# Ecogenomics/CheckM

Measured on NVIDIA H100. Metric: genomes/hour, higher is better.
Workload: dtype int16 (SSV) / u8 (MSV) / int16 (Viterbi) / f32 (Forward, domain definition)

## Files before the change

checkm_b200/csrc/fwdback_blk.cuh:

```cuda
#pragma once
#include "device_utils.cuh"
#include "engine.hpp"
#include "fwdback.cuh"

namespace ckm {

constexpr int BLK_LOOKAHEAD_MAXQ = 16;

template <int Q, bool TSMEM>
struct BlkModel {
  int M;
  const float *rfb;
  const float4 *tsm;
  float4 t0[TSMEM ? 1 : Q], t1[TSMEM ? 1 : Q];
  int lane;
  __device__ __forceinline__ float4 T0(int q) const { return TSMEM ? tsm[q * 32 + lane] : t0[TSMEM ? 0 : q]; }
  __device__ __forceinline__ float4 T1(int q) const { return TSMEM ? tsm[(Q + q) * 32 + lane] : t1[TSMEM ? 0 : q]; }
};

template <int Q, bool TSMEM>
__device__ __forceinline__ void blk_model_load(BlkModel<Q, TSMEM> &bm, const ModelScalars &ms, const float4 *tfb, const float *rfb,
                                               float4 *tsm, int lane) {
  bm.M = ms.M; bm.lane = lane;
  bm.rfb = rfb + ms.blk_off * 32 * KPAD + lane;
  bm.tsm = tsm;
  const float4 *src = tfb + ms.blk_off * 32 * 2;
  if (TSMEM) {
    __syncwarp();
    for (int q = 0; q < Q; ++q) { tsm[q * 32 + lane] = __ldg(src + (q * 32 + lane) * 2); tsm[(Q + q) * 32 + lane] = __ldg(src + (q * 32 + lane) * 2 + 1); }
    __syncwarp();
  } else {
#pragma unroll
    for (int q = 0; q < Q; ++q) { bm.t0[TSMEM ? 0 : q] = __ldg(src + (q * 32 + lane) * 2); bm.t1[TSMEM ? 0 : q] = __ldg(src + (q * 32 + lane) * 2 + 1); }
  }
}

template <int Q, bool TSMEM, bool FULL, bool STORE_D = true>
__device__ __forceinline__ float forward_blk(const BlkModel<Q, TSMEM> &bm, const uint8_t *__restrict__ res, int L, const Specials sp,
                                             float *xmx, float *full) {
  const int lane = bm.lane;
  float Mx[Q], Ix[Q], Dx[Q];
#pragma unroll
  for (int q = 0; q < Q; ++q) { Mx[q] = 0.0f; Ix[q] = 0.0f; Dx[q] = 0.0f; }
  if (FULL) {
#pragma unroll
    for (int z = 0; z < 3 * Q; ++z) full[z * 32 + lane] = 0.0f;
  }
  float xE = 0.0f, xN = 1.0f, xJ = 0.0f, xB = sp.nmove, xC = 0.0f, totscale = 0.0f;
  if (xmx != nullptr && lane == 0) { xmx[X_E] = xE; xmx[X_N] = xN; xmx[X_J] = xJ; xmx[X_B] = xB; xmx[X_C] = xC; xmx[X_SCALE] = 1.0f; }
  constexpr bool LA = (Q <= BLK_LOOKAHEAD_MAXQ);
  float ecur[Q];
  int xnext;
  if (LA) {
    const float *rp = bm.rfb + (size_t)((L >= 1) ? __ldg(res) : 0) * Q * 32;
#pragma unroll
    for (int q = 0; q < Q; ++q) ecur[q] = __ldg(rp + q * 32);
    xnext = (L >= 2) ? __ldg(res + 1) : 0;
  } else xnext = (L >= 1) ? __ldg(res) : 0;
  for (int i = 1; i <= L; ++i) {
    float enext[LA ? Q : 1];
    {
      const float *rp = bm.rfb + (size_t)xnext * Q * 32;
      if (LA) {
#pragma unroll
        for (int q = 0; q < Q; ++q) enext[LA ? q : 0] = __ldg(rp + q * 32);
        xnext = (i + 2 <= L) ? __ldg(res + i + 1) : 0;
      } else {
#pragma unroll
        for (int q = 0; q < Q; ++q) ecur[q] = __ldg(rp + q * 32);
        xnext = (i + 1 <= L) ? __ldg(res + i) : 0;
      }
    }
    float pm_in = __shfl_up_sync(0xffffffffu, Mx[Q - 1], 1), pi_in = __shfl_up_sync(0xffffffffu, Ix[Q - 1], 1), pd_in = __shfl_up_sync(0xffffffffu, Dx[Q - 1], 1);
    if (lane == 0) { pm_in = 0.0f; pi_in = 0.0f; pd_in = 0.0f; }
    float md[Q], esum = 0.0f;
#pragma unroll
    for (int q = Q - 1; q >= 0; --q) {
      const float4 t0 = bm.T0(q), t1 = bm.T1(q);
      const float pm = (q > 0) ? Mx[q - 1] : pm_in, pi = (q > 0) ? Ix[q - 1] : pi_in, pd = (q > 0) ? Dx[q - 1] : pd_in;
      float sv = xB * t0.x;
      sv += pm * t0.y;
      sv += pi * t0.z;
      sv += pd * t0.w;
      sv *= ecur[q];
      const float nI = Mx[q] * t1.y + Ix[q] * t1.z;
      md[q] = sv * t1.x;
      Mx[q] = sv; Ix[q] = nI;
      esum += sv;
    }
    float Bb = 0.0f, Tb = 1.0f;
#pragma unroll
    for (int q = 0; q < Q; ++q) { const float tdd = bm.T1(q).w; Bb = md[q] + Bb * tdd; Tb *= tdd; }
    float Bs = Bb, Ts = Tb;
#pragma unroll
    for (int o = 1; o < 32; o <<= 1) {
      const float Bl = __shfl_up_sync(0xffffffffu, Bs, o), Tl = __shfl_up_sync(0xffffffffu, Ts, o);
      if (lane >= o) { Bs = Bs + Bl * Ts; Ts = Ts * Tl; }
    }
    float d = __shfl_up_sync(0xffffffffu, Bs, 1);
    if (lane == 0) d = 0.0f;
#pragma unroll
    for (int q = 0; q < Q; ++q) {
      const bool in = (lane * Q + q + 1) <= bm.M;
      Dx[q] = in ? d : 0.0f;
      esum += Dx[q];
      d = md[q] + d * bm.T1(q).w;
    }
    xE = warp_sum_float(esum);
    xN = xN * sp.nloop;
    xC = (xC * sp.nloop) + (xE * sp.emove);
    xJ = (xJ * sp.nloop) + (xE * sp.eloop);
    xB = (xJ * sp.nmove) + (xN * sp.nmove);
    float scale = 1.0f;
    if (xE > 1.0e4f) {
      scale = xE;
      const float inv = __fdiv_rn(1.0f, xE);
      xN = __fdiv_rn(xN, xE); xC = __fdiv_rn(xC, xE); xJ = __fdiv_rn(xJ, xE); xB = __fdiv_rn(xB, xE);
#pragma unroll
      for (int q = 0; q < Q; ++q) { Mx[q] *= inv; Dx[q] *= inv; Ix[q] *= inv; }
      totscale += (float)log((double)xE);
      xE = 1.0f;
    }
    if (FULL) {
      float *fr = full + (size_t)i * 3 * Q * 32 + lane;
#pragma unroll
      for (int q = 0; q < Q; ++q) { fr[q * 32] = Mx[q]; if (STORE_D) fr[(Q + q) * 32] = Dx[q]; fr[(2 * Q + q) * 32] = Ix[q]; }
    }
    if (xmx != nullptr && lane == 0) {
      float *xr = xmx + (size_t)i * X_NX;
      xr[X_E] = xE; xr[X_N] = xN; xr[X_J] = xJ; xr[X_B] = xB; xr[X_C] = xC; xr[X_SCALE] = scale;
    }
    if (LA) {
#pragma unroll
      for (int q = 0; q < Q; ++q) ecur[q] = enext[LA ? q : 0];
    }
  }
  return totscale + (float)log((double)(xC * sp.nmove));
}

__device__ __forceinline__ void prefetch_l2(const void *p) { asm volatile("prefetch.global.L2 [%0];" ::"l"(p)); }
template <int Q, bool TSMEM, int MODE>
__device__ __forceinline__ void backward_blk(const BlkModel<Q, TSMEM> &bm, const uint8_t *__restrict__ res, int L, const Specials sp,
                                             const float *fxmx, float *bxmx, float *full) {
  const int lane = bm.lane, M = bm.M;
  float Mx[Q], Ix[Q], Dx[Q];
#pragma unroll
  for (int q = 0; q < Q; ++q) { Mx[q] = 0.0f; Ix[q] = 0.0f; Dx[q] = 0.0f; }
  float xC = 0.0f, xE = 0.0f, xJ = 0.0f, xN = 0.0f, xB = 0.0f;
  constexpr bool LA = (Q <= BLK_LOOKAHEAD_MAXQ);
  float ecur[Q];
#pragma unroll
  for (int q = 0; q < Q; ++q) ecur[q] = 0.0f;
  int xnext = (L >= 1) ? __ldg(res + L - 1) : 0;
  for (int i = L; i >= 0; --i) {
    float enext[LA ? Q : 1];
    if (LA) {
      const float *rp = bm.rfb + (size_t)xnext * Q * 32;
#pragma unroll
      for (int q = 0; q < Q; ++q) enext[LA ? q : 0] = __ldg(rp + q * 32);
      xnext = (i >= 2) ? __ldg(res + i - 2) : 0;
    } else if (i < L) {
      const float *rp = bm.rfb + (size_t)xnext * Q * 32;
#pragma unroll
      for (int q = 0; q < Q; ++q) ecur[q] = __ldg(rp + q * 32);
      xnext = (i >= 1) ? __ldg(res + i - 1) : 0;
    }
    if (MODE == 2 && i >= 3) {
      const float *fr = full + (size_t)(i - 2) * 3 * Q * 32;
      if (lane < Q) { prefetch_l2(fr + lane * 32); prefetch_l2(fr + (2 * Q + lane) * 32); }
    }
    float em[Q];
    if (i == L) {
      xC = sp.nmove; xE = xC * sp.emove; xB = 0.0f; xJ = 0.0f; xN = 0.0f;
#pragma unroll
      for (int q = 0; q < Q; ++q) em[q] = 0.0f;
    } else {
      float part = 0.0f;
#pragma unroll
      for (int q = 0; q < Q; ++q) { em[q] = Mx[q] * ecur[q]; part += em[q] * bm.T0(q).x; }
      xB = warp_sum_float(part);
      xC = xC * sp.nloop;
      xJ = (xB * sp.nmove) + (xJ * sp.nloop);
      xN = (xB * sp.nmove) + (xN * sp.nloop);
      xE = (xC * sp.emove) + (xJ * sp.eloop);
    }
    const float s = (i >= 1) ? fxmx[(size_t)i * X_NX + X_SCALE] : 1.0f;
    if (i >= 1) {
      const float inv = (s > 1.0f) ? __fdiv_rn(1.0f, s) : 1.0f;
      float em_next = __shfl_down_sync(0xffffffffu, em[0], 1);
      float4 tn_next;
      {
        const float4 mine = bm.T0(0);
        tn_next.x = 0.0f;
        tn_next.y = __shfl_down_sync(0xffffffffu, mine.y, 1); tn_next.z = __shfl_down_sync(0xffffffffu, mine.z, 1); tn_next.w = __shfl_down_sync(0xffffffffu, mine.w, 1);
      }
      if (lane == 31) { em_next = 0.0f; tn_next.y = 0.0f; tn_next.z = 0.0f; tn_next.w = 0.0f; }
      float cb[Q];
      float Bb = 0.0f, Tb = 1.0f;
#pragma unroll
      for (int q = Q - 1; q >= 0; --q) {
        const int k = lane * Q + q + 1;
        const float mnext = (q < Q - 1) ? em[q + 1] : em_next;
        const float tdm = (q < Q - 1) ? bm.T0(q + 1).w : tn_next.w;
        const bool in = (k <= M);
        cb[q] = in ? (xE + ((k < M) ? mnext * tdm : 0.0f)) : 0.0f;
        const float tdd = in ? bm.T1(q).w : 0.0f;
        Bb = cb[q] + Bb * tdd; Tb *= tdd;
      }
      float Bs = Bb, Ts = Tb;
#pragma unroll
      for (int o = 1; o < 32; o <<= 1) {
        const float Br = __shfl_down_sync(0xffffffffu, Bs, o), Tr = __shfl_down_sync(0xffffffffu, Ts, o);
        if (lane + o < 32) { Bs = Bs + Br * Ts; Ts = Ts * Tr; }
      }
      float dnext = __shfl_down_sync(0xffffffffu, Bs, 1);
      if (lane == 31) dnext = 0.0f;
      float nM[Q], nI[Q], nD[Q];
#pragma unroll
      for (int q = Q - 1; q >= 0; --q) {
        const int k = lane * Q + q + 1;
        const bool in = (k <= M);
        const float4 t1 = bm.T1(q);
        const float mnext = (q < Q - 1) ? em[q + 1] : em_next;
        const float4 tn = (q < Q - 1) ? bm.T0(q + 1) : tn_next;
        const float tmm = (k < M) ? tn.y : 0.0f, tim = (k < M) ? tn.z : 0.0f;
        const float inext = (i < L) ? Ix[q] : 0.0f;
        const float dv = in ? (cb[q] + dnext * t1.w) : 0.0f;
        float mv = xE + mnext * tmm + inext * t1.y + dnext * t1.x;
        float iv = mnext * tim + inext * t1.z;
        if (!in) { mv = 0.0f; iv = 0.0f; }
        nM[q] = mv * inv; nI[q] = iv * inv; nD[q] = dv * inv;
        dnext = dv;
      }
#pragma unroll
      for (int q = 0; q < Q; ++q) { Mx[q] = nM[q]; Ix[q] = nI[q]; Dx[q] = nD[q]; }
      if (s > 1.0f) { xE = __fdiv_rn(xE, s); xN = __fdiv_rn(xN, s); xJ = __fdiv_rn(xJ, s); xB = __fdiv_rn(xB, s); xC = __fdiv_rn(xC, s); }
    } else {
      xC = 0.0f; xJ = 0.0f; xE = 0.0f;
#pragma unroll
      for (int q = 0; q < Q; ++q) { Mx[q] = 0.0f; Ix[q] = 0.0f; Dx[q] = 0.0f; }
    }
    if (MODE == 1) {
      float *fr = full + (size_t)i * 3 * Q * 32 + lane;
#pragma unroll
      for (int q = 0; q < Q; ++q) { fr[q * 32] = Mx[q]; fr[(Q + q) * 32] = Dx[q]; fr[(2 * Q + q) * 32] = Ix[q]; }
    }
    if (MODE == 2 && i >= 1) {
      float *fr = full + (size_t)i * 3 * Q * 32 + lane;
      float fm[Q], fi[Q];
#pragma unroll
      for (int q = 0; q < Q; ++q) { fm[q] = fr[q * 32]; fi[q] = fr[(2 * Q + q) * 32]; }
#pragma unroll
      for (int q = 0; q < Q; ++q) { fr[q * 32] = fm[q] * Mx[q]; fr[(2 * Q + q) * 32] = fi[q] * Ix[q]; }
    }
    if (bxmx != nullptr && lane == 0) {
      float *xr = bxmx + (size_t)i * X_NX;
      xr[X_E] = xE; xr[X_N] = xN; xr[X_J] = xJ; xr[X_B] = xB; xr[X_C] = xC; xr[X_SCALE] = s;
    }
    if (LA) {
#pragma unroll
      for (int q = 0; q < Q; ++q) ecur[q] = enext[LA ? q : 0];
    }
  }
}

}
```

checkm_b200/csrc/kernels_blk.cu:

```cuda
#include "engine.hpp"
#include "device_utils.cuh"
#include "stages.hpp"
#include "fwdback.cuh"
#include "fwdback_blk.cuh"
#include "domdef_common.cuh"

namespace ckm {

constexpr int BLK_WARPS = 4;

template <int Q> __host__ __device__ constexpr size_t blk_tsm_bytes() { return (size_t)Q * 32 * 2 * sizeof(float4); }

template <int Q, bool TSMEM>
__global__ void __launch_bounds__(BLK_WARPS * 32) fwd2_kernel(FilterParams p) {
  extern __shared__ __align__(16) uint8_t bsm[];
  const int lane = threadIdx.x & 31, warp = threadIdx.x >> 5;
  float4 *tsm = reinterpret_cast<float4 *>(bsm) + (size_t)warp * Q * 32 * 2;
  const int n = min(*p.in_count, p.in_cap);
  for (int c = blockIdx.x * BLK_WARPS + warp; c < n; c += gridDim.x * BLK_WARPS) {
    Candidate cd = p.in[c];
    const ModelScalars ms = p.ms[cd.model];
    if (ms.vq != Q) continue;
    const int s = cd.seq, L = p.len[s];
    BlkModel<Q, TSMEM> bm;
    blk_model_load<Q, TSMEM>(bm, ms, p.tfb, p.rfb, tsm, lane);
    const float fsc = forward_blk<Q, TSMEM, false>(bm, p.res + p.off[s], L, make_specials(L, true), nullptr, nullptr);
    cd.fwdsc = fsc;
    const float seq_score = __fdiv_rn(__fsub_rn(fsc, cd.filtersc), 0.69314718055994529f);
    const double P = exp_surv((double)seq_score, (double)ms.evparam[4], (double)ms.evparam[5]);
    cd.P = P;
    if (lane == 0) {
      if (p.dense_fwd != nullptr) p.dense_fwd[(int64_t)p.model_slot[cd.model] * p.nseq + s] = fsc;
      if (P <= p.F3) {
        const int pos = atomicAdd(p.out_count, 1);
        if (pos < p.out_cap) p.out[pos] = cd;
        if (p.dense_passed != nullptr) atomicOr_u8(p.dense_passed, (int64_t)p.model_slot[cd.model] * p.nseq + s, 8);
      }
    }
  }
}

template <int Q, bool TSMEM>
__global__ void __launch_bounds__(BLK_WARPS * 32) regions2_kernel(DomdefParams p) {
  extern __shared__ __align__(16) uint8_t bsm[];
  const int lane = threadIdx.x & 31, warp = threadIdx.x >> 5;
  float4 *tsm = reinterpret_cast<float4 *>(bsm) + (size_t)warp * Q * 32 * 2;
  for (int idx = p.pair_begin + blockIdx.x * BLK_WARPS + warp; idx < p.pair_end; idx += gridDim.x * BLK_WARPS) {
    const int pi = p.pair_order[idx];
    const PairWork pw = p.pairs[pi];
    const ModelScalars ms = p.ms[pw.model];
    if (ms.vq != Q) continue;
    const int L = pw.L;
    BlkModel<Q, TSMEM> bm;
    blk_model_load<Q, TSMEM>(bm, ms, p.tfb, p.rfb, tsm, lane);
    const uint8_t *res = p.res + p.off[pw.seq];
    const Specials sp = make_specials(L, true);
    float *xf = p.xf + pw.row_off * X_NX, *xb = p.xb + pw.row_off * X_NX;
    forward_blk<Q, TSMEM, false>(bm, res, L, sp, xf, nullptr);
    __syncwarp();
    backward_blk<Q, TSMEM, 0>(bm, res, L, sp, xf, xb, nullptr);
    __syncwarp();
    regions_tail(p, pi, L, sp, xf, xb, p.btot + pw.row_off, p.etot + pw.row_off, p.mocc + pw.row_off, p.n2sc + pw.row_off, lane);
    __syncwarp();
  }
}

template <int Q, bool TSMEM>
__global__ void __launch_bounds__(BLK_WARPS * 32) envelope2_kernel(DomdefParams p) {
  extern __shared__ __align__(16) uint8_t bsm[];
  const int lane = threadIdx.x & 31, warp = threadIdx.x >> 5;
  float4 *tsm = reinterpret_cast<float4 *>(bsm) + (size_t)warp * Q * 32 * 2;
  float *null2 = reinterpret_cast<float *>(bsm + (TSMEM ? BLK_WARPS * blk_tsm_bytes<Q>() : 0)) + warp * 32;
  constexpr int QW = Q * 32;
  for (int idx = p.env_begin + blockIdx.x * BLK_WARPS + warp; idx < p.env_end; idx += gridDim.x * BLK_WARPS) {
    const int ei = p.env_order[idx];
    const Envelope env = p.envs[ei];
    const PairWork pw = p.pairs[env.pair];
    const ModelScalars ms = p.ms[pw.model];
    if (ms.vq != Q) continue;
    BlkModel<Q, TSMEM> bm;
    blk_model_load<Q, TSMEM>(bm, ms, p.tfb, p.rfb, tsm, lane);
    const int M = ms.M, Ld = env.j - env.i + 1;
    const uint8_t *res = p.res + p.off[pw.seq] + (env.i - 1);
    const Specials sp = make_specials(pw.L, false);
    const int64_t mat = (int64_t)(Ld + 1) * 3 * QW;
    float *F = p.scratch + env.scratch_off, *Bm = F;
    float *xf = F + mat, *xb = xf + (int64_t)(Ld + 1) * X_NX, *pps = xb + (int64_t)(Ld + 1) * X_NX;
    float *xo = xf;
    float *n2sc = p.n2sc + pw.row_off;
    const float envsc = forward_blk<Q, TSMEM, true, false>(bm, res, Ld, sp, xf, F);
    __syncwarp();
    backward_blk<Q, TSMEM, 2>(bm, res, Ld, sp, xf, xb, F);
    __syncwarp();
    const float scaleproduct = __fdiv_rn(1.0f, xb[X_N]);
    float em[Q], ein[Q];
#pragma unroll
    for (int q = 0; q < Q; ++q) { em[q] = 0.0f; ein[q] = 0.0f; }
    for (int r = 1; r <= Ld; ++r) {
      if (r + 2 <= Ld && lane < Q) {
        const float *fn = F + (int64_t)(r + 2) * 3 * QW;
        prefetch_l2(fn + lane * 32); prefetch_l2(fn + (2 * Q + lane) * 32);
      }
      const float totr = scaleproduct * xf[(int64_t)r * X_NX + X_SCALE];
      const float *fr = F + (int64_t)r * 3 * QW + lane;
      float vm[Q], vi[Q];
#pragma unroll
      for (int q = 0; q < Q; ++q) { vm[q] = fr[q * 32]; vi[q] = fr[(2 * Q + q) * 32]; }
#pragma unroll
      for (int q = 0; q < Q; ++q) {
        const float pm = vm[q] * totr, pi = vi[q] * totr;
        em[q] = (r == 1) ? pm : em[q] + pm;
        ein[q] = (r == 1) ? pi : ein[q] + pi;
      }
    }
    for (int r = lane; r <= Ld; r += 32) {
      float pn = 0.f, pj = 0.f, pc = 0.f;
      if (r >= 1) {
        const float *f0 = xf + (int64_t)(r - 1) * X_NX, *b1 = xb + (int64_t)r * X_NX;
        pn = f0[X_N] * b1[X_N] * sp.nloop * scaleproduct;
        pj = f0[X_J] * b1[X_J] * sp.nloop * scaleproduct;
        pc = f0[X_C] * b1[X_C] * sp.nloop * scaleproduct;
      }
      pps[r * 3 + 0] = pn; pps[r * 3 + 1] = pj; pps[r * 3 + 2] = pc;
    }
    __syncwarp();
    const bool range_err = isinf(scaleproduct);
    if (!range_err && !env.null2_done) {
      float xn = 0.f, xc = 0.f, xj = 0.f;
      if (lane == 0) {
        xn = pps[3 + 0]; xj = pps[3 + 1]; xc = pps[3 + 2];
        for (int r = 2; r <= Ld; ++r) { xn += pps[r * 3 + 0]; xj += pps[r * 3 + 1]; xc += pps[r * 3 + 2]; }
      }
      const float norm = __fdiv_rn(1.0f, (float)Ld);
#pragma unroll
      for (int q = 0; q < Q; ++q) { em[q] *= norm; ein[q] *= norm; }
      xn = __shfl_sync(0xffffffffu, xn, 0) * norm; xc = __shfl_sync(0xffffffffu, xc, 0) * norm; xj = __shfl_sync(0xffffffffu, xj, 0) * norm;
      const float xfactor = xn + xc + xj;
      for (int x = 0; x < K; ++x) {
        const float *rp = bm.rfb + (size_t)x * QW;
        float part = 0.0f;
#pragma unroll
        for (int q = 0; q < Q; ++q) { part += em[q] * __ldg(rp + q * 32); part += ein[q]; }
        part = warp_sum_float(part);
        if (lane == 0) null2[x] = part + xfactor;
      }
      __syncwarp();
      if (lane == 0) {
        { float r = 0.f; r += null2[2]; r += null2[11]; null2[21] = __fdiv_rn(r, 2.0f); }
        { float r = 0.f; r += null2[7]; r += null2[9];  null2[22] = __fdiv_rn(r, 2.0f); }
        { float r = 0.f; r += null2[3]; r += null2[13]; null2[23] = __fdiv_rn(r, 2.0f); }
        null2[24] = null2[8]; null2[25] = null2[1];
        float rx = 0.f;
        for (int x = 0; x < K; ++x) rx += null2[x];
        null2[26] = __fdiv_rn(rx, 20.0f);
        null2[20] = 1.0f; null2[27] = 1.0f; null2[28] = 1.0f; null2[29] = 1.0f;
      }
      __syncwarp();
      if (lane < KPAD) null2[lane] = (float)log((double)null2[lane]);
      __syncwarp();
      for (int pos = env.i + lane; pos <= env.j; pos += 32) n2sc[pos] = null2[res[pos - env.i]];
      __syncwarp();
    }
    float oasc = 0.0f;
    const float NINF = -INFINITY;
    if (!range_err) {
      float oM[Q], oI[Q], oD[Q];
#pragma unroll
      for (int q = 0; q < Q; ++q) { oM[q] = NINF; oI[q] = NINF; oD[q] = NINF; }
#pragma unroll
      for (int z = 0; z < 3 * Q; ++z) Bm[z * 32 + lane] = NINF;
      float oE = NINF, oN = 0.0f, oJ = NINF, oC = NINF, oB = (sp.nmove > 0.0f) ? 0.0f : NINF;
      if (lane == 0) { xo[X_E] = oE; xo[X_N] = oN; xo[X_J] = oJ; xo[X_B] = oB; xo[X_C] = oC; }
      for (int r = 1; r <= Ld; ++r) {
        if (r + 2 <= Ld && lane < Q) {
          const float *fn = F + (int64_t)(r + 2) * 3 * QW;
          prefetch_l2(fn + lane * 32); prefetch_l2(fn + (2 * Q + lane) * 32);
        }
        const float totr = scaleproduct * xf[(int64_t)r * X_NX + X_SCALE];
        const float *ppr = F + (int64_t)r * 3 * QW + lane;
        float *orow = Bm + (int64_t)r * 3 * QW + lane;
        float ppm[Q], ppi[Q];
#pragma unroll
        for (int q = 0; q < Q; ++q) { ppm[q] = ppr[q * 32]; ppi[q] = ppr[(2 * Q + q) * 32]; }
        float pm_in = __shfl_up_sync(0xffffffffu, oM[Q - 1], 1), pi_in = __shfl_up_sync(0xffffffffu, oI[Q - 1], 1), pd_in = __shfl_up_sync(0xffffffffu, oD[Q - 1], 1);
        if (lane == 0) { pm_in = NINF; pi_in = NINF; pd_in = NINF; }
        float a[Q]; bool ps[Q];
        float emax = NINF;
#pragma unroll
        for (int q = Q - 1; q >= 0; --q) {
          const float4 t0 = bm.T0(q), t1 = bm.T1(q);
          const bool in = (lane * Q + q + 1) <= M;
          const float pm = (q > 0) ? oM[q - 1] : pm_in, pi = (q > 0) ? oI[q - 1] : pi_in, pd = (q > 0) ? oD[q - 1] : pd_in;
          float sv = (t0.x > 0.0f) ? oB : 0.0f;
          sv = fmaxf(sv, (t0.y > 0.0f) ? pm : 0.0f);
          sv = fmaxf(sv, (t0.z > 0.0f) ? pi : 0.0f);
          sv = fmaxf(sv, (t0.w > 0.0f) ? pd : 0.0f);
          sv += ppm[q] * totr;
          if (!in) sv = NINF;
          const float nI = in ? fmaxf((t1.y > 0.0f) ? oM[q] : 0.0f, (t1.z > 0.0f) ? oI[q] : 0.0f) + ppi[q] * totr : NINF;
          a[q] = (t1.x > 0.0f) ? sv : 0.0f;
          ps[q] = (t1.w > 0.0f);
          if (!in) { a[q] = NINF; ps[q] = true; }
          if (!ps[q]) a[q] = fmaxf(a[q], 0.0f);
          oM[q] = sv; oI[q] = nI;
          emax = fmaxf(emax, sv);
        }
        float A = NINF; bool pass = true;
#pragma unroll
        for (int q = 0; q < Q; ++q) { if (ps[q]) { A = fmaxf(a[q], A); } else { A = a[q]; pass = false; } }
        float As = A; bool Ps = pass;
#pragma unroll
        for (int o = 1; o < 32; o <<= 1) {
          const float Al = __shfl_up_sync(0xffffffffu, As, o);
          const int pl = __shfl_up_sync(0xffffffffu, (int)Ps, o);
          if (lane >= o && Ps) { As = fmaxf(As, Al); Ps = (pl != 0); }
        }
        float d = __shfl_up_sync(0xffffffffu, As, 1);
        if (lane == 0) d = NINF;
#pragma unroll
        for (int q = 0; q < Q; ++q) {
          const bool in = (lane * Q + q + 1) <= M;
          oD[q] = in ? d : NINF;
          emax = fmaxf(emax, oD[q]);
          d = ps[q] ? fmaxf(a[q], d) : a[q];
        }
#pragma unroll
        for (int o = 16; o > 0; o >>= 1) emax = fmaxf(emax, __shfl_xor_sync(0xffffffffu, emax, o));
        oE = emax;
        const float ppn = pps[r * 3 + 0], ppj = pps[r * 3 + 1], ppc = pps[r * 3 + 2];
        float t1s = (sp.nloop == 0.0f) ? FLT_MIN_F : 1.0f, t2s = (sp.eloop == 0.0f) ? FLT_MIN_F : 1.0f;
        oJ = fmaxf(t1s * (oJ + ppj), t2s * oE);
        t2s = (sp.emove == 0.0f) ? FLT_MIN_F : 1.0f;
        oC = fmaxf(t1s * (oC + ppc), t2s * oE);
        oN = t1s * (oN + ppn);
        t1s = (sp.nmove == 0.0f) ? FLT_MIN_F : 1.0f;
        oB = fmaxf(t1s * oN, t1s * oJ);
#pragma unroll
        for (int q = 0; q < Q; ++q) { orow[q * 32] = oM[q]; orow[(Q + q) * 32] = oD[q]; orow[(2 * Q + q) * 32] = oI[q]; }
        if (lane == 0) { float *xr = xo + (int64_t)r * X_NX; xr[X_E] = oE; xr[X_N] = oN; xr[X_J] = oJ; xr[X_B] = oB; xr[X_C] = oC; }
      }
      oasc = oC;
    }
    __syncwarp();
    bool ok = !range_err;
    int hmmfrom = 0, hmmto = 0, sqfrom = 0, sqto = 0;
#define CELL(row, st, k) Bm[((int64_t)(row) * 3 + (st)) * QW + (((k) - 1) % Q) * 32 + ((k) - 1) / Q]
#define TT0(k) (__ldg(p.tfb + ms.blk_off * 64 + ((((k) - 1) % Q) * 32 + ((k) - 1) / Q) * 2))
#define TT1(k) (__ldg(p.tfb + ms.blk_off * 64 + ((((k) - 1) % Q) * 32 + ((k) - 1) / Q) * 2 + 1))
    if (ok) {
      int i = Ld, k = 0, s0 = ST_C, s1 = -1;
      int firstMi = 0, firstMk = 0, lastMi = 0, lastMk = 0; bool have_last = false;
      int guard = 0;
      while (s0 != ST_S && ok) {
        if (++guard > 4 * (Ld + M) + 16) { ok = false; break; }
        const float *xc = xo + (int64_t)i * X_NX;
        if (s0 == ST_M) {
          const float4 t0 = TT0(k);
          float path[4];
          path[0] = (t0.y > 0.0f && k > 1) ? CELL(i - 1, 0, k - 1) : -INFINITY;
          path[1] = (t0.z > 0.0f && k > 1) ? CELL(i - 1, 2, k - 1) : -INFINITY;
          path[2] = (t0.w > 0.0f && k > 1) ? CELL(i - 1, 1, k - 1) : -INFINITY;
          path[3] = (t0.x > 0.0f) ? xo[(int64_t)(i - 1) * X_NX + X_B] : -INFINITY;
          int best = 0;
          for (int z = 1; z < 4; ++z) if (path[z] > path[best]) best = z;
          s1 = (best == 0) ? ST_M : (best == 1) ? ST_I : (best == 2) ? ST_D : ST_B;
          k--; i--;
        } else if (s0 == ST_D) {
          const float4 t1 = TT1(k - 1);
          const float a = (t1.x > 0.0f) ? CELL(i, 0, k - 1) : -INFINITY, b = (t1.w > 0.0f) ? CELL(i, 1, k - 1) : -INFINITY;
          s1 = (a >= b) ? ST_M : ST_D; k--;
        } else if (s0 == ST_I) {
          const float4 t1 = TT1(k);
          const float a = (t1.y > 0.0f) ? CELL(i - 1, 0, k) : -INFINITY, b = (t1.z > 0.0f) ? CELL(i - 1, 2, k) : -INFINITY;
          s1 = (a >= b) ? ST_M : ST_I; i--;
        } else if (s0 == ST_N) {
          s1 = (i == 0) ? ST_S : ST_N;
        } else if (s0 == ST_C) {
          const float t1s = (sp.nloop == 0.0f) ? FLT_MIN_F : 1.0f, t2s = (sp.emove == 0.0f) ? FLT_MIN_F : 1.0f;
          const float a = (i > 0) ? t1s * (xo[(int64_t)(i - 1) * X_NX + X_C] + pps[i * 3 + 2]) : -INFINITY, b = t2s * xc[X_E];
          s1 = (a > b) ? ST_C : ST_E;
        } else if (s0 == ST_J) {
          const float t1s = (sp.nloop == 0.0f) ? FLT_MIN_F : 1.0f, t2s = (sp.eloop == 0.0f) ? FLT_MIN_F : 1.0f;
          const float a = (i > 0) ? t1s * (xo[(int64_t)(i - 1) * X_NX + X_J] + pps[i * 3 + 1]) : -INFINITY, b = t2s * xc[X_E];
          s1 = (a > b) ? ST_J : ST_E;
        } else if (s0 == ST_E) {
          const float *dpc = Bm + (int64_t)i * 3 * QW + lane;
          float bmv = -INFINITY; int bk = -1, bdk = -1; float bd = -INFINITY;
#pragma unroll
          for (int q = 0; q < Q; ++q) {
            const int kk = lane * Q + q + 1;
            if (kk <= M) {
              const float v = dpc[q * 32]; if (v >= bmv) { bmv = v; bk = kk; }
              const float w = dpc[(Q + q) * 32]; if (w > bd) { bd = w; bdk = kk; }
            }
          }
#pragma unroll
          for (int o = 16; o > 0; o >>= 1) {
            const float om = __shfl_xor_sync(0xffffffffu, bmv, o); const int ok2 = __shfl_xor_sync(0xffffffffu, bk, o);
            if (om > bmv || (om == bmv && ok2 > bk)) { bmv = om; bk = ok2; }
            const float od = __shfl_xor_sync(0xffffffffu, bd, o); const int odk = __shfl_xor_sync(0xffffffffu, bdk, o);
            if (od > bd || (od == bd && odk >= 0 && (bdk < 0 || odk < bdk))) { bd = od; bdk = odk; }
          }
          if (bd > bmv) { s1 = ST_D; k = bdk; } else { s1 = ST_M; k = bk; }
          if (k < 1) { ok = false; break; }
        } else if (s0 == ST_B) {
          const float t1s = (sp.nmove == 0.0f) ? FLT_MIN_F : 1.0f;
          s1 = (t1s * xc[X_N] > t1s * xc[X_J]) ? ST_N : ST_J;
        } else { ok = false; break; }
        if (s1 == ST_M) {
          if (!have_last || s0 == ST_E) { lastMi = i; lastMk = k; have_last = true; }
          firstMi = i; firstMk = k;
          if (p.trace != nullptr && lane == 0) p.trace[pw.row_off + env.i - 1 + i] = k;
        } else if (s1 == ST_I) {
          if (p.trace != nullptr && lane == 0) p.trace[pw.row_off + env.i - 1 + i] = -k;
        }
        if ((s1 == ST_N || s1 == ST_J || s1 == ST_C) && s1 == s0) i--;
        s0 = s1;
      }
      if (!have_last) ok = false;
      hmmfrom = firstMk; hmmto = lastMk; sqfrom = firstMi + env.i - 1; sqto = lastMi + env.i - 1;
    }
#undef CELL
#undef TT0
#undef TT1
    if (lane == 0) {
      DomainOut out;
      out.pair = env.pair; out.ienv = env.i; out.jenv = env.j;
      float domcorrection = 0.0f;
      for (int pos = env.i; pos <= env.j; ++pos) domcorrection += n2sc[pos];
      out.ok = ok ? 1 : 0;
      out.envsc = envsc; out.oasc = oasc; out.domcorrection = domcorrection;
      out.hmmfrom = hmmfrom; out.hmmto = hmmto; out.sqfrom = sqfrom; out.sqto = sqto;
      out.bitscore = 0.f; out.dombias = 0.f; out.pad = 0.f; out.lnP = 0.0;
      p.doms[env.slot] = out;
    }
    __syncwarp();
  }
}

template <int Q, bool TSMEM, class P, class KF>
static int launch_one(KF kern, const P &p, int grid, size_t extra, cudaStream_t st, const char *what) {
  const size_t smem = (TSMEM ? BLK_WARPS * blk_tsm_bytes<Q>() : 0) + extra;
  if (smem > 48 * 1024) {
    cudaError_t e = cudaFuncSetAttribute(kern, cudaFuncAttributeMaxDynamicSharedMemorySize, (int)smem);
    if (e != cudaSuccess) return cuda_fail(e, what);
  }
  kern<<<grid, BLK_WARPS * 32, smem, st>>>(p);
  cudaError_t e = cudaGetLastError();
  return e == cudaSuccess ? CKM_OK : cuda_fail(e, what);
}

#define CKM_CLASS_SWITCH(KERN, EXTRA, WHAT)                                                              \
  switch (cls) {                                                                                        \
    case 0: return launch_one<2, false>(KERN<2, false>, p, grid, EXTRA, st, WHAT);                      \
    case 1: return launch_one<4, false>(KERN<4, false>, p, grid, EXTRA, st, WHAT);                      \
    case 2: return launch_one<6, false>(KERN<6, false>, p, grid, EXTRA, st, WHAT);                      \
    case 3: return launch_one<8, false>(KERN<8, false>, p, grid, EXTRA, st, WHAT);                      \
    case 4: return launch_one<12, true>(KERN<12, true>, p, grid, EXTRA, st, WHAT);                      \
    case 5: return launch_one<16, true>(KERN<16, true>, p, grid, EXTRA, st, WHAT);                      \
    case 6: return launch_one<20, true>(KERN<20, true>, p, grid, EXTRA, st, WHAT);                      \
    case 7: return launch_one<24, true>(KERN<24, true>, p, grid, EXTRA, st, WHAT);                      \
    case 8: return launch_one<28, true>(KERN<28, true>, p, grid, EXTRA, st, WHAT);                      \
    case 9: return launch_one<32, true>(KERN<32, true>, p, grid, EXTRA, st, WHAT);                      \
  }                                                                                                     \
  set_error(WHAT ": bad class"); return CKM_EINVAL;

int launch_fwd2(const FilterParams &p, int cls, int grid, cudaStream_t st) { CKM_CLASS_SWITCH(fwd2_kernel, 0, "fwd2_kernel") }
int launch_regions2(const DomdefParams &p, int cls, int grid, cudaStream_t st) { CKM_CLASS_SWITCH(regions2_kernel, 0, "regions2_kernel") }
int launch_envelopes2(const DomdefParams &p, int cls, int grid, cudaStream_t st) {
  const size_t extra = BLK_WARPS * 32 * sizeof(float);
  CKM_CLASS_SWITCH(envelope2_kernel, extra, "envelope2_kernel")
}

}
```

checkm_b200/csrc/kernels_ensemble.cu:

```cuda
#include <algorithm>
#include <vector>
#include "engine.hpp"
#include "device_utils.cuh"
#include "stages.hpp"
#include "fwdback.cuh"
#include "pool.hpp"

namespace ckm {

constexpr int NSAMPLES = 200;

struct EnsembleParams {
  DomdefParams d;
  const Region *regions; const int32_t *multi_idx; int32_t nmulti;
  const int64_t *scratch_off;
  float *scratch;
  const EnsembleCaps *caps;
  const int64_t *env_off;
  Envelope *env_out; int32_t *env_count;
  int32_t *need;
};

enum { ST_M = 1, ST_D, ST_I, ST_S, ST_N, ST_B, ST_E, ST_C, ST_T, ST_J };

struct Lcg { uint32_t x; };
__device__ __forceinline__ uint32_t mix3(uint32_t a, uint32_t b, uint32_t c) {
  a -= b; a -= c; a ^= (c >> 13);
  b -= c; b -= a; b ^= (a << 8);
  c -= a; c -= b; c ^= (b >> 13);
  a -= b; a -= c; a ^= (c >> 12);
  b -= c; b -= a; b ^= (a << 16);
  c -= a; c -= b; c ^= (b >> 5);
  a -= b; a -= c; a ^= (c >> 3);
  b -= c; b -= a; b ^= (a << 10);
  c -= a; c -= b; c ^= (b >> 15);
  return c;
}
__device__ __forceinline__ double lcg_random(Lcg &r) { r.x *= 69069u; r.x += 1u; return (double)r.x / 4294967296.0; }

__device__ __forceinline__ int fchoose(Lcg &rng, float *pth, int N) {
  float sum = 0.0f;
  for (int i = 0; i < N; ++i) sum = __fadd_rn(sum, pth[i]);
  if (sum != 0.0f) { const float s = (float)(1.0 / (double)sum); for (int i = 0; i < N; ++i) pth[i] = __fmul_rn(pth[i], s); }
  else for (int i = 0; i < N; ++i) pth[i] = __fdiv_rn(1.0f, (float)N);
  const float roll = (float)lcg_random(rng);
  sum = 0.0f;
  for (int i = 0; i < N; ++i) { sum = __fadd_rn(sum, pth[i]); if (roll < sum) return i; }
  int i;
  int guard = 0;
  do { i = (int)(lcg_random(rng) * N); } while (pth[i] == 0.0f && ++guard < 64);
  return i;
}

__device__ __forceinline__ bool sp_link(const int *a, const int *b) {
  int nov = min(a[2], b[2]) - max(a[1], b[1]) + 1;
  int n = min(a[2] - a[1] + 1, b[2] - b[1] + 1);
  if ((float)nov / (float)n < 0.8f) return false;
  nov = min(a[4], b[4]) - max(a[3], b[3]);
  n = min(a[4] - a[3] + 1, b[4] - b[3] + 1);
  if ((float)nov / (float)n < 0.8f) return false;
  if (abs((a[1] - a[3]) - (b[1] - b[3])) > 4) return false;
  if (abs((a[2] - a[4]) - (b[2] - b[4])) > 4) return false;
  return true;
}

__global__ void __launch_bounds__(FWD_WARPS * 32) ensemble_kernel(EnsembleParams ep) {
  extern __shared__ __align__(16) uint8_t smem[];
  const DomdefParams &p = ep.d;
  const int lane = threadIdx.x & 31, warp = threadIdx.x >> 5;
  float *rowM = reinterpret_cast<float *>(smem) + (size_t)warp * 3 * p.row_elems;
  float *rowI = rowM + p.row_elems, *rowD = rowI + p.row_elems;
  for (int ri = blockIdx.x * FWD_WARPS + warp; ri < ep.nmulti; ri += gridDim.x * FWD_WARPS) {
    const Region reg = ep.regions[ep.multi_idx[ri]];
    const PairWork pw = p.pairs[reg.pair];
    const ModelScalars ms = p.ms[pw.model];
    FwdModel fm;
    fm.M = ms.M; fm.Mpad = ms.Mpad;
    fm.rfv = p.rfv + (int64_t)ms.off_cells * KPAD;
    fm.tfv = reinterpret_cast<const float4 *>(p.tfv + (int64_t)ms.off_cells * T_N);
    const int M = fm.M, Mpad = fm.Mpad, Lr = reg.j - reg.i + 1;
    const int Q = max(2, (M + 3) / 4);
    const uint8_t *res = p.res + p.off[pw.seq] + (reg.i - 1);
    const Specials sp = make_specials(pw.L, true);
    float *F = ep.scratch + ep.scratch_off[ri];
    float *xf = F + (int64_t)(Lr + 1) * 3 * Mpad;
    float *acc = xf + (int64_t)(Lr + 1) * X_NX, *val = acc + (Lr + 1);
    const EnsembleCaps cap = ep.caps[ri];
    const int SPCAP = cap.segments, TRCAP = cap.trace_segments, MAXENV = cap.envelopes;
    int *spb = reinterpret_cast<int *>(val + (Lr + 1));
    int *label = spb + (int64_t)SPCAP * 5;
    int *epc = label + (int64_t)3 * SPCAP;
    int *segbuf = epc + max(Lr, M) + 2;
    int most_in_trace = 0;
    float *n2sc = p.n2sc + pw.row_off;
    forward_rows<true, true>(fm, res, Lr, sp, rowM, rowI, rowD, lane, xf, F, 0, nullptr);
    for (int pos = lane; pos <= Lr; pos += 32) acc[pos] = 0.0f;
    __syncwarp();
    Lcg rng; rng.x = mix3(42u, 87654321u, 12345678u); if (rng.x == 0) rng.x = 42;
    uint32_t jA = 1u, jC = 0u;
    for (int z = 0; z <= lane; ++z) { jC = jC * 69069u + 1u; jA *= 69069u; }
    int nsp = 0;
    float *cm = rowM, *ci = rowI, *null2 = rowD;
    for (int t = 0; t < NSAMPLES; ++t) {
      for (int pos = lane; pos <= Lr; pos += 32) val[pos] = 1.0f;
      __syncwarp();
      int i = Lr, k = 0, s0 = ST_C, s1 = -1;
      int nseg = 0;
      int sqto = 0, hmmto = 0, sqfrom = 0, hmmfrom = 0, ldom = 0;
      bool in_dom = false, failed = false;
      long guard = 0;
      const long gmax = 8L * (Lr + 2) * (M + 2);
      while (s0 != ST_S) {
        if (++guard > gmax) { failed = true; break; }
        float pth[4];
        if (s0 == ST_M || s0 == ST_C || s0 == ST_J) {
          const bool isM = (s0 == ST_M);
          const int ii = i - lane, kk = k - lane;
          const bool valid = isM ? (ii >= 1 && kk >= 1) : (ii >= 0);
          float p0 = 0.f, p1 = 0.f, p2 = 0.f, p3 = 0.f;
          if (valid) {
            if (isM) {
              const float *dpp = F + (int64_t)(ii - 1) * 3 * Mpad;
              const float4 t0 = __ldg(fm.tfv + 2 * kk);
              p0 = __fmul_rn(xf[(int64_t)(ii - 1) * X_NX + X_B], t0.x);
              p1 = __fmul_rn(dpp[kk - 1], t0.y);
              p2 = __fmul_rn(dpp[2 * Mpad + kk - 1], t0.z);
              p3 = __fmul_rn(dpp[Mpad + kk - 1], t0.w);
            } else {
              const int XS = (s0 == ST_C) ? X_C : X_J;
              const float tmv = (s0 == ST_C) ? sp.emove : sp.eloop;
              p0 = (ii > 0) ? __fmul_rn(xf[(int64_t)(ii - 1) * X_NX + XS], sp.nloop) : 0.0f;
              p1 = __fmul_rn(__fmul_rn(xf[(int64_t)ii * X_NX + X_E], tmv), xf[(int64_t)ii * X_NX + X_SCALE]);
            }
          }
          const int np = isM ? 4 : 2;
          float sum = __fadd_rn(__fadd_rn(0.0f, p0), p1);
          if (isM) sum = __fadd_rn(__fadd_rn(sum, p2), p3);
          if (sum != 0.0f) { const float sc = (float)(1.0 / (double)sum); p0 = __fmul_rn(p0, sc); p1 = __fmul_rn(p1, sc); p2 = __fmul_rn(p2, sc); p3 = __fmul_rn(p3, sc); }
          else { const float u = __fdiv_rn(1.0f, (float)np); p0 = u; p1 = u; p2 = u; p3 = u; }
          const uint32_t xl = jA * rng.x + jC;
          const float roll = (float)((double)xl / 4294967296.0);
          const float c0 = __fadd_rn(0.0f, p0), c1 = __fadd_rn(c0, p1), c2 = __fadd_rn(c1, p2), c3 = __fadd_rn(c2, p3);
          int choice = -1;
          if (roll < c0) choice = 0; else if (roll < c1) choice = 1; else if (isM && roll < c2) choice = 2; else if (isM && roll < c3) choice = 3;
          const bool okl = valid && choice >= 0;
          const int stay = isM ? 1 : 0;
          const unsigned cont = __ballot_sync(0xffffffffu, okl && choice == stay);
          const int nlead = (cont == 0xffffffffu) ? 32 : (__ffs(~cont) - 1);
          const int okf = (nlead < 32) ? __shfl_sync(0xffffffffu, (int)okl, nlead & 31) : 0;
          const int cf = __shfl_sync(0xffffffffu, choice, nlead & 31);
          const int nproc = nlead + (okf ? 1 : 0);
          if (nproc > 0) {
            guard += nproc - 1;
            if (nlead > 0) {
              if (isM) {
                if (in_dom) {
                  if (sqto == 0) sqto = i - 1;
                  if (hmmto == 0) hmmto = k - 1;
                  sqfrom = i - nlead; hmmfrom = k - nlead; ldom += nlead;
                  if (lane < nlead) cm[k - lane - 1] += 1.0f;
                }
                k -= nlead;
              }
              i -= nlead;
            }
            rng.x = __shfl_sync(0xffffffffu, xl, nproc - 1);
            if (!okf) continue;
            if (isM) { s1 = (cf == 0) ? ST_B : (cf == 2) ? ST_I : ST_D; k--; i--; }
            else s1 = ST_E;
            goto step_done;
          }
        }
        if (s0 == ST_M) {
          const float *dpp = F + (int64_t)(i - 1) * 3 * Mpad;
          const float4 t0 = __ldg(fm.tfv + 2 * k);
          pth[0] = __fmul_rn(xf[(int64_t)(i - 1) * X_NX + X_B], t0.x);
          pth[1] = __fmul_rn(dpp[k - 1], t0.y);
          pth[2] = __fmul_rn(dpp[2 * Mpad + k - 1], t0.z);
          pth[3] = __fmul_rn(dpp[Mpad + k - 1], t0.w);
          const int c = fchoose(rng, pth, 4);
          s1 = (c == 0) ? ST_B : (c == 1) ? ST_M : (c == 2) ? ST_I : ST_D;
          k--; i--;
        } else if (s0 == ST_D) {
          const float *dpc = F + (int64_t)i * 3 * Mpad;
          const float4 t1 = __ldg(fm.tfv + 2 * (k - 1) + 1);
          pth[0] = __fmul_rn(dpc[k - 1], t1.x);
          pth[1] = __fmul_rn(dpc[Mpad + k - 1], t1.w);
          s1 = fchoose(rng, pth, 2) == 0 ? ST_M : ST_D; k--;
        } else if (s0 == ST_I) {
          const float *dpp = F + (int64_t)(i - 1) * 3 * Mpad;
          const float4 t1 = __ldg(fm.tfv + 2 * k + 1);
          pth[0] = __fmul_rn(dpp[k], t1.y);
          pth[1] = __fmul_rn(dpp[2 * Mpad + k], t1.z);
          s1 = fchoose(rng, pth, 2) == 0 ? ST_M : ST_I; i--;
        } else if (s0 == ST_N) {
          i = 0; s1 = ST_S;
        } else if (s0 == ST_C) {
          pth[0] = (i > 0) ? __fmul_rn(xf[(int64_t)(i - 1) * X_NX + X_C], sp.nloop) : 0.0f;
          pth[1] = __fmul_rn(__fmul_rn(xf[(int64_t)i * X_NX + X_E], sp.emove), xf[(int64_t)i * X_NX + X_SCALE]);
          s1 = fchoose(rng, pth, 2) == 0 ? ST_C : ST_E;
        } else if (s0 == ST_J) {
          pth[0] = (i > 0) ? __fmul_rn(xf[(int64_t)(i - 1) * X_NX + X_J], sp.nloop) : 0.0f;
          pth[1] = __fmul_rn(__fmul_rn(xf[(int64_t)i * X_NX + X_E], sp.eloop), xf[(int64_t)i * X_NX + X_SCALE]);
          s1 = fchoose(rng, pth, 2) == 0 ? ST_J : ST_E;
        } else if (s0 == ST_B) {
          pth[0] = __fmul_rn(xf[(int64_t)i * X_NX + X_N], sp.nmove);
          pth[1] = __fmul_rn(xf[(int64_t)i * X_NX + X_J], sp.nmove);
          s1 = fchoose(rng, pth, 2) == 0 ? ST_N : ST_J;
        } else if (s0 == ST_E) {
          const float *dpc = F + (int64_t)i * 3 * Mpad;
          const double roll = lcg_random(rng);
          const float norm = (float)(1.0 / (double)xf[(int64_t)i * X_NX + X_E]);
          const int nent = 8 * Q, per = (nent + 31) / 32;
          const int e0 = lane * per, e1 = min(nent, e0 + per);
          double part = 0.0;
          for (int e = e0; e < e1; ++e) {
            const int q = e >> 3, r = e & 3, isd = (e >> 2) & 1, kk = r * Q + q + 1;
            const float v = (kk <= M) ? __fmul_rn(dpc[isd * Mpad + kk], norm) : 0.0f;
            part += (double)v;
          }
          double incl = part;
#pragma unroll
          for (int o = 1; o < 32; o <<= 1) { const double up = __shfl_up_sync(0xffffffffu, incl, o); if (lane >= o) incl += up; }
          const unsigned hitmask = __ballot_sync(0xffffffffu, roll < incl && e1 > e0);
          int sel = -1;
          if (hitmask != 0u) {
            const int owner = __ffs(hitmask) - 1;
            if (lane == owner) {
              double sum = incl - part;
              for (int e = e0; e < e1; ++e) {
                const int q = e >> 3, r = e & 3, isd = (e >> 2) & 1, kk = r * Q + q + 1;
                const float v = (kk <= M) ? __fmul_rn(dpc[isd * Mpad + kk], norm) : 0.0f;
                sum += (double)v;
                if (roll < sum) { sel = e; break; }
              }
              if (sel < 0) sel = e1 - 1;
            }
            sel = __shfl_sync(0xffffffffu, sel, owner);
          }
          if (sel < 0) { failed = true; break; }
          { const int q = sel >> 3, r = sel & 3, isd = (sel >> 2) & 1; k = r * Q + q + 1; s1 = isd ? ST_D : ST_M; }
          if (k > M) { failed = true; break; }
          in_dom = true; sqto = 0; hmmto = 0; sqfrom = 0; hmmfrom = 0; ldom = 0;
          for (int kk = lane; kk <= M; kk += 32) { cm[kk] = 0.0f; ci[kk] = 0.0f; }
          __syncwarp();
        } else { failed = true; break; }
      step_done:
        if (in_dom) {
          if (s1 == ST_M) {
            if (sqto == 0) sqto = i;
            if (hmmto == 0) hmmto = k;
            sqfrom = i; hmmfrom = k; ldom++;
            if (lane == 0) cm[k] += 1.0f;
          } else if (s1 == ST_I) {
            ldom++;
            if (lane == 0) ci[k] += 1.0f;
          } else if (s1 == ST_D) {
            if (hmmto == 0) hmmto = k;
            hmmfrom = k;
          } else if (s1 == ST_B) {
            __syncwarp();
            const float nrm = __fdiv_rn(1.0f, (float)ldom);
            for (int kk = lane + 1; kk <= M; kk += 32) { cm[kk] *= nrm; ci[kk] *= nrm; }
            __syncwarp();
            for (int x = 0; x < K; ++x) {
              const float *rp = fm.rfv + (int64_t)x * Mpad;
              float part = 0.0f;
              for (int kk = lane + 1; kk <= M; kk += 32) { part += cm[kk] * __ldg(rp + kk); part += ci[kk]; }
              part = warp_sum_float(part);
              if (lane == 0) null2[x] = part;
            }
            __syncwarp();
            if (lane == 0) {
              { float r = 0.f; r += null2[2]; r += null2[11]; null2[21] = __fdiv_rn(r, 2.0f); }
              { float r = 0.f; r += null2[7]; r += null2[9];  null2[22] = __fdiv_rn(r, 2.0f); }
              { float r = 0.f; r += null2[3]; r += null2[13]; null2[23] = __fdiv_rn(r, 2.0f); }
              null2[24] = null2[8]; null2[25] = null2[1];
              float rx = 0.f;
              for (int x = 0; x < K; ++x) rx += null2[x];
              null2[26] = __fdiv_rn(rx, 20.0f);
              null2[20] = 1.0f; null2[27] = 1.0f; null2[28] = 1.0f; null2[29] = 1.0f;
            }
            __syncwarp();
            for (int pos = sqfrom + 1 + lane; pos <= sqto; pos += 32) val[pos] = null2[res[pos - 1]];
            if (lane == 0 && nseg < TRCAP) { segbuf[nseg * 4 + 0] = sqfrom; segbuf[nseg * 4 + 1] = sqto; segbuf[nseg * 4 + 2] = hmmfrom; segbuf[nseg * 4 + 3] = hmmto; }
            nseg++;
            in_dom = false;
            __syncwarp();
          }
        }
        if ((s1 == ST_N || s1 == ST_J || s1 == ST_C) && s1 == s0) i--;
        s0 = s1;
      }
      __syncwarp();
      if (failed) continue;
      for (int pos = 1 + lane; pos <= Lr; pos += 32) acc[pos] += val[pos];
      if (lane == 0) {
        most_in_trace = max(most_in_trace, nseg);
        for (int z = min(nseg, TRCAP) - 1; z >= 0; --z) {
          if (nsp + 0 < SPCAP) {
            int *e = spb + nsp * 5;
            e[0] = t; e[1] = segbuf[z * 4 + 0] + reg.i - 1; e[2] = segbuf[z * 4 + 1] + reg.i - 1; e[3] = segbuf[z * 4 + 2]; e[4] = segbuf[z * 4 + 3];
          }
          nsp++;
        }
        nsp += max(nseg - TRCAP, 0);
      }
      nsp = __shfl_sync(0xffffffffu, nsp, 0);
      __syncwarp();
    }
    most_in_trace = __shfl_sync(0xffffffffu, most_in_trace, 0);
    const int nsp_all = nsp + 0;
    const bool sp_overflow = nsp > SPCAP || most_in_trace > TRCAP;
    nsp = min(nsp, SPCAP);
    for (int pos = reg.i + lane; pos <= reg.j; pos += 32) n2sc[pos] = (float)log((double)__fdiv_rn(acc[pos - reg.i + 1], (float)NSAMPLES));
    int *avail = label, *stack = label + SPCAP, *assign = label + 2 * SPCAP;
    for (int h = lane; h < nsp; h += 32) avail[h] = h;
    __syncwarp();
    int na = nsp, nb = 0, nc = 0;
    while (na > 0) {
      int v = avail[na - 1]; na--;
      stack[nb++] = v;
      while (nb > 0) {
        v = stack[--nb];
        assign[v] = nc;
        for (int base = na - 1; base >= 0; base -= 32) {
          const int pos = base - lane;
          bool linked = false;
          if (pos >= 0) linked = sp_link(spb + v * 5, spb + avail[pos] * 5);
          unsigned mask = __ballot_sync(0xffffffffu, linked);
          while (mask != 0u) {
            const int l = __ffs(mask) - 1;
            mask &= mask - 1;
            const int pz = base - l;
            const int w = avail[pz];
            avail[pz] = avail[na - 1];
            na--;
            stack[nb++] = w;
          }
          __syncwarp();
        }
      }
      nc++;
    }
    __syncwarp();
    if (lane == 0) {
      int nout = 0;
      Envelope *eo = ep.env_out + ep.env_off[ri];
      for (int c = 0; c < nc; ++c) {
        int idx_of_last = -1, ninc = 0;
        for (int h = 0; h < nsp; ++h) if (assign[h] == c) { if (spb[h * 5] != idx_of_last) ninc++; idx_of_last = spb[h * 5]; }
        if ((float)ninc / (float)NSAMPLES < 0.25f) continue;
        int imin = 1 << 30, jmin = 1 << 30, imax = 0, jmax = 0;
        for (int h = 0; h < nsp; ++h) if (assign[h] == c) {
          imin = min(imin, spb[h * 5 + 1]); imax = max(imax, spb[h * 5 + 1]);
          jmin = min(jmin, spb[h * 5 + 2]); jmax = max(jmax, spb[h * 5 + 2]);
        }
        int cmv, best_i, best_j;
        for (int z = 0; z <= imax - imin; ++z) epc[z] = 0;
        for (int h = 0; h < nsp; ++h) if (assign[h] == c) epc[spb[h * 5 + 1] - imin]++;
        for (cmv = 0, best_i = imin; best_i <= imax; ++best_i) { cmv += epc[best_i - imin]; if ((float)cmv / (float)ninc >= 0.02f) break; }
        for (int z = 0; z <= jmax - jmin; ++z) epc[z] = 0;
        for (int h = 0; h < nsp; ++h) if (assign[h] == c) epc[spb[h * 5 + 2] - jmin]++;
        for (cmv = 0, best_j = jmax; best_j >= jmin; --best_j) { cmv += epc[best_j - jmin]; if ((float)cmv / (float)ninc >= 0.02f) break; }
        if (best_i > best_j) continue;
        if (nout < MAXENV) { eo[nout].pair = reg.pair; eo[nout].i = best_i; eo[nout].j = best_j; eo[nout].null2_done = 1; eo[nout].scratch_off = 0; eo[nout].slot = 0; eo[nout].pad = 0; }
        nout++;
      }
      const int nsig = nout;
      nout = min(nout, MAXENV);
      for (int a = 1; a < nout; ++a) { Envelope v = eo[a]; int b = a - 1; while (b >= 0 && eo[b].i > v.i) { eo[b + 1] = eo[b]; --b; } eo[b + 1] = v; }
      ep.env_count[ri] = (sp_overflow || nsig > MAXENV) ? -1 : nsig;
      ep.need[ri * 3 + 0] = nsp_all; ep.need[ri * 3 + 1] = most_in_trace; ep.need[ri * 3 + 2] = nsig;
    }
    __syncwarp();
  }
}

struct EnsembleJob {
  DevBuf b_regs, b_idx, b_off, b_scr, b_env, b_cnt, b_caps, b_eoff, b_need;
  std::vector<int64_t> off, env_off;
  std::vector<Envelope> envs;
  std::vector<int32_t> cnt, need;
  std::vector<EnsembleCaps> caps;
  int nm = 0;
};

int ensembles_launch(ckm_engine *e, const ckm_models *m, DomdefParams &p, const std::vector<PairWork> &pairs,
                     const std::vector<Region> &regs, const std::vector<int> &multi_idx, const std::vector<EnsembleCaps> &caps,
                     cudaStream_t st, EnsembleJob **job_out) {
  EnsembleJob *job = new EnsembleJob();
  *job_out = job;
  const int nm = job->nm = (int)multi_idx.size();
  job->off.resize(nm); job->env_off.resize(nm); job->caps = caps;
  int64_t tot = 0, nenv = 0;
  for (int i = 0; i < nm; ++i) {
    const Region &r = regs[multi_idx[i]];
    const int64_t Lr = r.j - r.i + 1, M = m->models[pairs[r.pair].model].M, Mpad = ((M + 1) + 31) / 32 * 32 + 32;
    job->off[i] = tot;
    tot += (Lr + 1) * 3 * Mpad + (Lr + 1) * X_NX + 2 * (Lr + 1) + (int64_t)caps[i].segments * 8 + std::max(Lr, M) + 2 + (int64_t)caps[i].trace_segments * 4 + 64;
    tot = (tot + 63) / 64 * 64;
    job->env_off[i] = nenv;
    nenv += caps[i].envelopes;
  }
  int rc;
  if ((rc = job->b_regs.alloc(sizeof(Region) * regs.size())) || (rc = job->b_idx.alloc(sizeof(int32_t) * nm)) || (rc = job->b_off.alloc(sizeof(int64_t) * nm)) ||
      (rc = job->b_scr.alloc(sizeof(float) * (size_t)tot)) || (rc = job->b_env.alloc(sizeof(Envelope) * (size_t)nenv)) || (rc = job->b_cnt.alloc(sizeof(int32_t) * nm)) ||
      (rc = job->b_caps.alloc(sizeof(EnsembleCaps) * nm)) || (rc = job->b_eoff.alloc(sizeof(int64_t) * nm)) || (rc = job->b_need.alloc(sizeof(int32_t) * 3 * nm))) return rc;
  CKM_CUDA(cudaMemcpyAsync(job->b_regs.p, regs.data(), sizeof(Region) * regs.size(), cudaMemcpyHostToDevice, st));
  CKM_CUDA(cudaMemcpyAsync(job->b_idx.p, multi_idx.data(), sizeof(int32_t) * nm, cudaMemcpyHostToDevice, st));
  CKM_CUDA(cudaMemcpyAsync(job->b_off.p, job->off.data(), sizeof(int64_t) * nm, cudaMemcpyHostToDevice, st));
  CKM_CUDA(cudaMemcpyAsync(job->b_caps.p, job->caps.data(), sizeof(EnsembleCaps) * nm, cudaMemcpyHostToDevice, st));
  CKM_CUDA(cudaMemcpyAsync(job->b_eoff.p, job->env_off.data(), sizeof(int64_t) * nm, cudaMemcpyHostToDevice, st));
  CKM_CUDA(cudaMemsetAsync(job->b_cnt.p, 0, sizeof(int32_t) * nm, st));
  CKM_CUDA(cudaMemsetAsync(job->b_need.p, 0, sizeof(int32_t) * 3 * nm, st));
  CKM_CUDA(cudaMemsetAsync(job->b_env.p, 0, sizeof(Envelope) * (size_t)nenv, st));
  EnsembleParams ep;
  ep.d = p; ep.regions = job->b_regs.as<Region>(); ep.multi_idx = job->b_idx.as<int32_t>(); ep.nmulti = nm;
  ep.scratch_off = job->b_off.as<int64_t>(); ep.scratch = job->b_scr.as<float>(); ep.env_out = job->b_env.as<Envelope>(); ep.env_count = job->b_cnt.as<int32_t>();
  ep.caps = job->b_caps.as<EnsembleCaps>(); ep.env_off = job->b_eoff.as<int64_t>(); ep.need = job->b_need.as<int32_t>();
  const size_t smem = (size_t)FWD_WARPS * 3 * p.row_elems * sizeof(float);
  CKM_CUDA(cudaFuncSetAttribute(ensemble_kernel, cudaFuncAttributeMaxDynamicSharedMemorySize, (int)smem));
  const int grid = std::min(e->prop.multiProcessorCount * 4, (nm + FWD_WARPS - 1) / FWD_WARPS);
  ensemble_kernel<<<grid, FWD_WARPS * 32, smem, st>>>(ep);
  CKM_CUDA(cudaGetLastError());
  e->stats.kernel_launches++;
  job->envs.resize((size_t)nenv);
  job->cnt.resize(nm); job->need.resize((size_t)3 * nm);
  CKM_CUDA(cudaMemcpyAsync(job->envs.data(), job->b_env.p, sizeof(Envelope) * job->envs.size(), cudaMemcpyDeviceToHost, st));
  CKM_CUDA(cudaMemcpyAsync(job->cnt.data(), job->b_cnt.p, sizeof(int32_t) * nm, cudaMemcpyDeviceToHost, st));
  CKM_CUDA(cudaMemcpyAsync(job->need.data(), job->b_need.p, sizeof(int32_t) * 3 * nm, cudaMemcpyDeviceToHost, st));
  return CKM_OK;
}

int ensembles_collect(EnsembleJob *job, cudaStream_t st, std::vector<std::vector<Envelope>> &out, std::vector<EnsembleCaps> &grow, int *n_over) {
  cudaError_t err = cudaStreamSynchronize(st);
  *n_over = 0;
  if (err == cudaSuccess) {
    out.assign((size_t)job->nm, {});
    grow.assign((size_t)job->nm, EnsembleCaps{0, 0, 0});
    for (int i = 0; i < job->nm; ++i) {
      if (job->cnt[i] < 0) {
        const EnsembleCaps &c = job->caps[i];
        const bool traces_cut = job->need[3 * i] > c.segments || job->need[3 * i + 1] > c.trace_segments;
        EnsembleCaps g = c;
        g.segments = std::max(c.segments, job->need[3 * i] + 64);
        g.trace_segments = std::max(c.trace_segments, job->need[3 * i + 1] + 8);
        g.envelopes = std::max(c.envelopes, traces_cut ? std::max(2 * job->need[3 * i + 2], job->need[3 * i + 1] + 8) : job->need[3 * i + 2]);
        grow[i] = g;
        ++*n_over;
        continue;
      }
      for (int c = 0; c < job->cnt[i]; ++c) out[i].push_back(job->envs[(size_t)job->env_off[i] + c]);
    }
  }
  delete job;
  if (err != cudaSuccess) return cuda_fail(err, "ensemble job");
  return CKM_OK;
}
void ensembles_abandon(EnsembleJob *job, cudaStream_t st) { if (job) { cudaStreamSynchronize(st); delete job; } }

}
```

checkm_b200/csrc/search.cu:

```cuda
#include <algorithm>
#include <atomic>
#include <chrono>
#include <cstdio>
#include <cmath>
#include <cstdlib>
#include <cstring>
#include <memory>
#include <vector>
#include "engine.hpp"
#include "stages.hpp"
#include "pool.hpp"

using namespace ckm;

namespace ckm {

std::atomic<int> g_live_engines{0};
thread_local ckm_engine *g_pool_engine = nullptr;
thread_local int g_pool_next = 0;
constexpr int X_NX_HOST = 6;
struct EnsembleJob;
int ensembles_launch(ckm_engine *e, const ckm_models *m, DomdefParams &p, const std::vector<PairWork> &pairs,
                     const std::vector<Region> &regs, const std::vector<int> &multi_idx, const std::vector<EnsembleCaps> &caps,
                     cudaStream_t st, EnsembleJob **job_out);
int ensembles_collect(EnsembleJob *job, cudaStream_t st, std::vector<std::vector<Envelope>> &out, std::vector<EnsembleCaps> &grow, int *n_over);
void ensembles_abandon(EnsembleJob *job, cudaStream_t st);
enum { CTR_UNIT4 = 0, CTR_UNIT8, CTR_UNIT16, CTR_UNIT32, CTR_CAND, CTR_MSV, CTR_BIAS, CTR_VIT, CTR_FWD, CTR_ENV, CTR_DOM, CTR_VREDO, CTR_SSVRES, CTR_VWORK = 16 , CTR_N = 32 };
enum { EV_SSV = 0, EV_MSV, EV_BIAS, EV_VIT, EV_FWD, EV_CASCADE_END, EV_DOMDEF, EV_END, EV_CALL };

static int64_t env_scratch_budget() {
  if (const char *v = std::getenv("CKM_ENV_SCRATCH_MB")) {
    char *end = nullptr;
    const long long mb = std::strtoll(v, &end, 10);
    if (end != v && *end == '\0' && mb > 0) return (int64_t)std::min<long long>(mb, (long long)1 << 30) * ((int64_t)1 << 20) / (int64_t)sizeof(float);
  }
  size_t free_b = 0, total_b = 0;
  cudaMemGetInfo(&free_b, &total_b);
  const size_t neng = (size_t)std::max(1, g_live_engines.load());
  return (int64_t)std::min<size_t>(total_b * 4 / 10 / neng, (size_t)56 << 30) / (int64_t)sizeof(float);
}
struct SearchKnobs { bool blk, vitp, ssv_resolve, trace; int ens_first; int64_t env_budget; };
static SearchKnobs read_knobs(bool envelopes) {
  auto starts = [](const char *name, char c) { const char *v = std::getenv(name); return v != nullptr && v[0] == c; };
  SearchKnobs k;
  k.blk = !starts("CKM_BLK", '0');
  k.vitp = k.blk && !starts("CKM_VITP", '0');
  k.ssv_resolve = !starts("CKM_SSV_RESOLVE", '0');
  k.trace = starts("CKM_TRACE", '1');
  const char *ens = std::getenv("CKM_ENS_FIRST");
  k.ens_first = ens == nullptr ? -1 : (ens[0] == '0' ? 0 : 1);
  k.env_budget = envelopes ? env_scratch_budget() : 0;
  return k;
}
struct Trace {
  bool on; std::chrono::steady_clock::time_point t0, last;
  explicit Trace(bool on_) : on(on_) { t0 = last = std::chrono::steady_clock::now(); }
  void mark(const char *what) {
    if (!on) return;
    const auto now = std::chrono::steady_clock::now();
    std::fprintf(stderr, "[ckm trace] %-28s +%8.3f ms  (%9.3f)\n", what, std::chrono::duration<double, std::milli>(now - last).count(),
                 std::chrono::duration<double, std::milli>(now - t0).count());
    last = now;
  }
};

static int vq_of(int M) { return (M <= 64) ? 2 : (M <= 128) ? 4 : (M <= 192) ? 6 : (M <= 256) ? 8 : (M <= 384) ? 12 : (M <= 512) ? 16 : (M <= 640) ? 20 : (M <= 768) ? 24 : (M <= 896) ? 28 : (M <= 1024) ? 32 : 0; }
static int cls_of(int M, bool use_blk) {
  if (!use_blk) return N_BLK_CLASSES;
  const int q = vq_of(M);
  for (int c = 0; c < N_BLK_CLASSES; ++c) if (BLK_Q[c] == q) return c;
  return N_BLK_CLASSES;
}

static int fan_out(ckm_engine *e) {
  CKM_CUDA(cudaEventRecord(e->fan_ev, e->stream));
  for (auto &s : e->cls) CKM_CUDA(cudaStreamWaitEvent(s, e->fan_ev, 0));
  return CKM_OK;
}
static int fan_in(ckm_engine *e) {
  for (int c = 0; c < ckm_engine::NCLS; ++c) {
    CKM_CUDA(cudaEventRecord(e->cls_ev[c], e->cls[c]));
    CKM_CUDA(cudaStreamWaitEvent(e->stream, e->cls_ev[c], 0));
  }
  return CKM_OK;
}

template <class P> static int per_class(ckm_engine *e, const P &p, int (*blocked)(const P &, int, int, cudaStream_t), int blk_per_sm,
                                        int (*unblocked)(const P &, int, cudaStream_t), int per_sm, bool widest_first = false) {
  const int nsm = e->prop.multiProcessorCount;
  int rc;
  if ((rc = fan_out(e))) return rc;
  for (int i = 0; i < ckm_engine::NCLS; ++i) {
    const int c = widest_first ? ckm_engine::NCLS - 1 - i : i;
    if (c == N_BLK_CLASSES) rc = unblocked ? unblocked(p, nsm * per_sm, e->cls[c]) : CKM_OK;
    else rc = p.use_blk ? blocked(p, c, nsm * blk_per_sm, e->cls[c]) : CKM_OK;
    if (rc) return rc;
  }
  return fan_in(e);
}
template <class Launch> static int launch_class_runs(ckm_engine *e, const std::vector<int32_t> &order, const std::vector<int8_t> &cls, size_t b0, size_t b1, Launch launch) {
  const int nsm = e->prop.multiProcessorCount;
  int rc;
  if ((rc = fan_out(e))) return rc;
  while (b0 < b1) {
    size_t r1 = b0; const int c = cls[order[b0]];
    while (r1 < b1 && cls[order[r1]] == c) ++r1;
    const int cnt = (int)(r1 - b0);
    const int grid = c < N_BLK_CLASSES ? std::min(nsm * 8, (cnt + 3) / 4) : std::min(nsm * 4, (cnt + FWD_WARPS - 1) / FWD_WARPS);
    if ((rc = launch(c, (int32_t)b0, (int32_t)r1, grid, e->cls[c]))) return rc;
    e->stats.kernel_launches++;
    b0 = r1;
  }
  return CKM_OK;
}

struct ActiveMasks { DevBuf tile_active, model_active, model_slot; bool all_active = true; };
static FilterParams filter_params(const ckm_models *m, const ckm_seqdb *db, ActiveMasks &am) {
  FilterParams p{};
  p.res = db->d_res; p.off = db->d_off; p.len = db->d_len; p.lenA = db->d_lenA; p.lenB = db->d_lenB; p.tmove_w = db->d_tmove_w;
  p.ms = m->d_scalars; p.bias_eo = m->d_bias_eo; p.rwv = m->d_rwv; p.twv = m->d_twv; p.rfv = m->d_rfv; p.tfv = m->d_tfv;
  p.twb = m->d_twb; p.rwb = m->d_rwb; p.tfb = m->d_tfb; p.rfb = m->d_rfb; p.twp = m->d_twp; p.rwp = m->d_rwp;
  p.row_elems = ((m->maxM + 31) / 32) * 32 + 64;
  p.F1 = 0.02; p.F2 = 1e-3; p.F3 = 1e-5;
  p.model_slot = am.model_slot.as<int32_t>(); p.nseq = db->nseq;
  return p;
}

static DomdefParams domdef_params(const ckm_models *m, const ckm_seqdb *db, const SearchKnobs &k) {
  DomdefParams p{};
  p.res = db->d_res; p.off = db->d_off; p.nullsc = db->d_nullsc; p.ms = m->d_scalars; p.rfv = m->d_rfv; p.tfv = m->d_tfv;
  p.row_elems = ((m->maxM + 31) / 32) * 32 + 64;
  p.tfb = m->d_tfb; p.rfb = m->d_rfb; p.use_blk = k.blk ? 1 : 0;
  return p;
}
static void fill_filter_stats(ckm_engine *e, int64_t n_pairs, const int32_t *ctr, unsigned long long cells, int stages) {
  ckm_stats &s = e->stats;
  s.n_pairs = n_pairs; s.n_cells = (int64_t)cells;
  s.n_ssv_cand = (int64_t)ctr[CTR_CAND] + ctr[CTR_SSVRES]; s.n_msv_exact = ctr[CTR_CAND]; s.n_past_msv = ctr[CTR_MSV]; s.n_past_bias = ctr[CTR_BIAS];
  s.n_past_vit = ctr[CTR_VIT]; s.n_past_fwd = ctr[CTR_FWD]; s.n_vit_redo = ctr[CTR_VREDO];
  float *ms[] = {&s.ms_ssv, &s.ms_msv, &s.ms_bias, &s.ms_vit, &s.ms_fwd};
  for (int i = 0; i < stages; ++i) cudaEventElapsedTime(ms[i], e->ev[EV_SSV + i], e->ev[EV_SSV + i + 1]);
}
static std::vector<float> &logsum_table() {
  static std::vector<float> t = [] {
    std::vector<float> v(16000);
    for (int i = 0; i < 16000; ++i) v[i] = (float)std::log(1.0 + std::exp((double)-i / 1000.0));
    return v;
  }();
  return t;
}

static int build_masks(const ckm_models *m, const ckm_seqdb *db, const int32_t *model_idx, int32_t nmodels,
                       const int64_t *bin_model_offsets, ActiveMasks &am, std::vector<int32_t> &slot_of_model, cudaStream_t st) {
  const int ndb = (int)m->models.size(), nbins = db->nbins, ntiles = (int)m->tiles.size();
  slot_of_model.assign(ndb, -1);
  bool all = (bin_model_offsets == nullptr) && (model_idx == nullptr || nmodels == ndb);
  if (model_idx == nullptr) { for (int i = 0; i < ndb; ++i) slot_of_model[i] = i; }
  else if (bin_model_offsets == nullptr) {
    for (int i = 0; i < nmodels; ++i) {
      if (model_idx[i] < 0 || model_idx[i] >= ndb) { set_error("model index out of range"); return CKM_EINVAL; }
      if (slot_of_model[model_idx[i]] >= 0) { set_error("duplicate model index in query list"); return CKM_EINVAL; }
      slot_of_model[model_idx[i]] = i;
    }
    if (all) for (int i = 0; i < ndb; ++i) if (slot_of_model[i] < 0) all = false;
  }
  am.all_active = all;
  int rc;
  if ((rc = am.model_slot.alloc(sizeof(int32_t) * ndb))) return rc;
  CKM_CUDA(cudaMemcpyAsync(am.model_slot.p, slot_of_model.data(), sizeof(int32_t) * ndb, cudaMemcpyHostToDevice, st));
  if (all) return CKM_OK;
  std::vector<uint8_t> ma((size_t)nbins * ndb, 0), ta((size_t)nbins * ntiles, 0);
  for (int b = 0; b < nbins; ++b) {
    if (bin_model_offsets == nullptr) {
      for (int i = 0; i < nmodels; ++i) ma[(size_t)b * ndb + model_idx[i]] = 1;
    } else {
      for (int64_t i = bin_model_offsets[b]; i < bin_model_offsets[b + 1]; ++i) {
        if (model_idx[i] < 0 || model_idx[i] >= ndb) { set_error("model index out of range"); return CKM_EINVAL; }
        if (ma[(size_t)b * ndb + model_idx[i]]) { set_error("duplicate model index in the query list of bin " + std::to_string(b)); return CKM_EINVAL; }
        ma[(size_t)b * ndb + model_idx[i]] = 1;
      }
    }
    for (int t = 0; t < ntiles; ++t) {
      const TileDesc &td = m->tiles[t];
      uint8_t any = 0;
      for (int j = 0; j < td.nmodels; ++j) any |= ma[(size_t)b * ndb + m->tile_models[td.first_model + j].model];
      ta[(size_t)b * ntiles + t] = any;
    }
  }
  if ((rc = am.model_active.alloc(ma.size()))) return rc;
  if ((rc = am.tile_active.alloc(ta.size()))) return rc;
  CKM_CUDA(cudaMemcpyAsync(am.model_active.p, ma.data(), ma.size(), cudaMemcpyHostToDevice, st));
  CKM_CUDA(cudaMemcpyAsync(am.tile_active.p, ta.data(), ta.size(), cudaMemcpyHostToDevice, st));
  CKM_CUDA(cudaStreamSynchronize(st));
  return CKM_OK;
}
struct Stage1 {
  DevBuf cand, pass, bnd, glist, cells;
  int32_t cand_cap = 0, pass_cap = 0;
};
constexpr int64_t QUEUE_MAX = (int64_t)1 << 30;
constexpr int QUEUE_ATTEMPTS = 3;
static int32_t queue_cap(int64_t n_pairs, int64_t divisor, int attempt) {
  int64_t want = n_pairs / divisor + 65536;
  for (int a = 0; a < attempt && want < n_pairs; ++a) want *= 8;
  return (int32_t)std::min<int64_t>(std::min<int64_t>(n_pairs, QUEUE_MAX), std::max<int64_t>((int64_t)1 << 16, want));
}

static int run_stage1(ckm_engine *e, const SearchKnobs &k, const ckm_models *m, const ckm_seqdb *db, ActiveMasks &am, int64_t n_pairs,
                      Stage1 &s1, int32_t *xj_dense, int attempt = 0) {
  cudaStream_t st = e->stream;
  int rc;
  s1.cand_cap = queue_cap(n_pairs, 6, attempt);
  const int64_t n_bypass = (int64_t)m->ssv_bypass.size() * db->nseq;
  s1.cand_cap = (int32_t)std::min<int64_t>(QUEUE_MAX, (int64_t)s1.cand_cap + n_bypass);
  s1.pass_cap = queue_cap(n_pairs, 12, attempt);
  if ((rc = s1.cand.alloc(sizeof(int2) * (size_t)s1.cand_cap))) return rc;
  if ((rc = s1.pass.alloc(sizeof(Candidate) * (size_t)s1.pass_cap))) return rc;
  if ((rc = s1.cells.alloc(sizeof(unsigned long long)))) return rc;
  CKM_CUDA(cudaMemsetAsync(e->d_counters, 0, CTR_N * sizeof(int32_t), st));
  CKM_CUDA(cudaMemsetAsync(s1.cells.p, 0, sizeof(unsigned long long), st));
  const int nsm = e->prop.multiProcessorCount;
  bool need_bnd = false;
  for (int nt : m->chain_ntiles) need_bnd |= (nt > 1);
  const int64_t bnd_stride = ((int64_t)db->maxL + 31) / 16 * 16;
  if (need_bnd) { if ((rc = s1.bnd.alloc((size_t)nsm * SSV_WARPS_HOST * 2 * bnd_stride * sizeof(int16_t)))) return rc; }
  std::vector<int32_t> gl[4];
  for (size_t g = 0; g < m->groups.size(); ++g) gl[m->groups[g].J == 4 ? 0 : (m->groups[g].J == 8 ? 1 : (m->groups[g].J == 16 ? 2 : 3))].push_back((int32_t)g);
  std::vector<int32_t> flat;
  size_t goff[4];
  for (int c = 0; c < 4; ++c) { goff[c] = flat.size(); flat.insert(flat.end(), gl[c].begin(), gl[c].end()); }
  if ((rc = s1.glist.alloc(sizeof(int32_t) * std::max<size_t>(flat.size(), 1)))) return rc;
  if (!flat.empty()) CKM_CUDA(cudaMemcpyAsync(s1.glist.p, flat.data(), sizeof(int32_t) * flat.size(), cudaMemcpyHostToDevice, st));
  CKM_CUDA(cudaStreamSynchronize(st));

  CKM_CUDA(cudaEventRecord(e->ev[EV_SSV], st));
  SsvParams sp{};
  sp.res = db->d_res; sp.off = db->d_off; sp.len = db->d_len; sp.bin = db->d_bin;
  sp.msvB = db->d_msvB; sp.tjb = db->d_tjb; sp.order = db->d_order;
  sp.nseq = db->nseq; sp.seq_chunk = 128; sp.nchunks = (db->nseq + sp.seq_chunk - 1) / sp.seq_chunk;
  sp.groups = m->d_groups; sp.tiles = m->d_tiles; sp.tile_models = m->d_tile_models; sp.tile_blob = m->d_tile_blob;
  sp.chain_first_tile = m->d_chain_first_tile; sp.chain_ntiles = m->d_chain_ntiles;
  sp.tile_active = am.all_active ? nullptr : am.tile_active.as<uint8_t>();
  sp.model_active = am.all_active ? nullptr : am.model_active.as<uint8_t>();
  sp.ntiles = (int32_t)m->tiles.size(); sp.nmodels = (int32_t)m->models.size();
  sp.cand = s1.cand.as<int2>(); sp.cand_count = e->d_counters + CTR_CAND; sp.cand_cap = s1.cand_cap;
  sp.bnd = need_bnd ? s1.bnd.as<int16_t>() : nullptr; sp.bnd_stride = bnd_stride;
  sp.cells = s1.cells.as<unsigned long long>();
  sp.resolve = k.ssv_resolve ? 1 : 0;
  sp.ms = m->d_scalars; sp.nullsc = db->d_nullsc;
  sp.pass = s1.pass.as<Candidate>(); sp.pass_count = e->d_counters + CTR_MSV; sp.pass_cap = s1.pass_cap;
  sp.resolved_count = e->d_counters + CTR_SSVRES;
  sp.xj_dense = xj_dense; sp.model_slot = am.model_slot.as<int32_t>();
  sp.F1 = 0.02;
  const int Js[4] = {4, 8, 16, 32};
  for (int c = 0; c < 4; ++c) {
    if (gl[c].empty() || db->nseq == 0) continue;
    sp.group_list = s1.glist.as<int32_t>() + goff[c]; sp.ngroups = (int32_t)gl[c].size();
    sp.unit_counter = e->d_counters + CTR_UNIT4 + c;
    int64_t maxbytes = 0;
    for (int g : gl[c]) maxbytes = std::max<int64_t>(maxbytes, m->groups[g].table_bytes);
    const int64_t units = (int64_t)sp.ngroups * sp.nchunks;
    const int grid = (int)std::min<int64_t>(nsm, units);
    if ((rc = launch_ssv(Js[c], sp, grid, (size_t)maxbytes, st))) return rc;
    e->stats.kernel_launches++;
  }
  if (!m->ssv_bypass.empty()) {
    if ((rc = launch_ssv_bypass(m->d_ssv_bypass, (int32_t)m->ssv_bypass.size(), db->nseq, db->d_len, db->d_bin,
                                am.all_active ? nullptr : am.model_active.as<uint8_t>(), (int32_t)m->models.size(),
                                s1.cand.as<int2>(), e->d_counters + CTR_CAND, s1.cand_cap, st))) return rc;
    e->stats.kernel_launches++;
  }
  CKM_CUDA(cudaEventRecord(e->ev[EV_MSV], st));
  MsvParams p{};
  p.res = db->d_res; p.off = db->d_off; p.len = db->d_len; p.nullsc = db->d_nullsc; p.tjb = db->d_tjb;
  p.ms = m->d_scalars; p.rbv = m->d_rbv; p.rmb = m->d_rmb;
  p.cand = s1.cand.as<int2>(); p.cand_count = e->d_counters + CTR_CAND; p.cand_cap = s1.cand_cap;
  p.out = s1.pass.as<Candidate>(); p.out_count = e->d_counters + CTR_MSV; p.out_cap = s1.pass_cap;
  p.xj_dense = xj_dense; p.model_slot = am.model_slot.as<int32_t>(); p.nseq = db->nseq;
  p.row_bytes = (m->maxM + 2 + 15) / 16 * 16;
  p.F1 = 0.02;
  p.use_blk = k.blk ? 1 : 0;
  if ((rc = per_class(e, p, launch_msv2, 16, launch_msv_exact, 4))) return rc;
  e->stats.kernel_launches += 1 + (p.use_blk ? N_BLK_CLASSES : 0);
  CKM_CUDA(cudaEventRecord(e->ev[EV_BIAS], st));
  return CKM_OK;
}

static int run_viterbi(ckm_engine *e, const ckm_models *m, FilterParams &p, bool packed, DevBuf &grp) {
  int rc;
  if (packed) {
    const int nm = (int)m->models.size();
    const size_t nchunks = (size_t)p.in_cap / VITP_CHUNK + nm + 1;
    const size_t words = 4 * (size_t)nm + 16 + ((size_t)p.in_cap + 1) / 2 * 2;
    if ((rc = grp.alloc(sizeof(int32_t) * words + sizeof(int2) * nchunks))) return rc;
    int32_t *ws = grp.as<int32_t>();
    p.vit_cls_chunks = ws + 4 * (size_t)nm;
    p.vit_idx = p.vit_cls_chunks + 16;
    p.vit_chunks = reinterpret_cast<int2 *>(ws + words);
    p.vit_work = e->d_counters + CTR_VWORK;
    if ((rc = launch_vit_group(p, nm, ws, e->prop.multiProcessorCount * 8, e->stream))) return rc;
    if ((rc = per_class<FilterParams>(e, p, launch_vitp, 8, nullptr, 0))) return rc;
    e->stats.kernel_launches += 3;
    p.in = p.redo; p.in_count = p.redo_count; p.in_cap = p.redo_cap;
  }
  return per_class(e, p, launch_vit2, 8, launch_vit, 4);
}
struct Stage2 {
  DevBuf a, b, redo, vgrp;
  int32_t cap = 0;
};
static int run_stage2(ckm_engine *e, const SearchKnobs &k, const ckm_models *m, const ckm_seqdb *db, ActiveMasks &am, Stage1 &s1, Stage2 &s2,
                      float *d_filtersc, float *d_vit, float *d_fwd, uint8_t *d_passed) {
  cudaStream_t st = e->stream;
  int rc;
  s2.cap = s1.pass_cap;
  if ((rc = s2.a.alloc(sizeof(Candidate) * (size_t)s2.cap))) return rc;
  if ((rc = s2.b.alloc(sizeof(Candidate) * (size_t)s2.cap))) return rc;
  if ((rc = s2.redo.alloc(sizeof(Candidate) * (size_t)s2.cap))) return rc;
  const int nsm = e->prop.multiProcessorCount;
  FilterParams p = filter_params(m, db, am);
  p.redo = s2.redo.as<Candidate>(); p.redo_count = e->d_counters + CTR_VREDO; p.redo_cap = s2.cap;
  p.use_blk = k.blk ? 1 : 0;
  p.dense_filtersc = d_filtersc; p.dense_vit = d_vit; p.dense_fwd = d_fwd; p.dense_passed = d_passed;
  p.in = s1.pass.as<Candidate>(); p.in_count = e->d_counters + CTR_MSV; p.in_cap = s1.pass_cap;
  p.out = s2.a.as<Candidate>(); p.out_count = e->d_counters + CTR_BIAS; p.out_cap = s2.cap;
  if ((rc = launch_bias(p, nsm * 8, st))) return rc;
  CKM_CUDA(cudaEventRecord(e->ev[EV_VIT], st));
  p.in = s2.a.as<Candidate>(); p.in_count = e->d_counters + CTR_BIAS; p.in_cap = s2.cap;
  p.out = s2.b.as<Candidate>(); p.out_count = e->d_counters + CTR_VIT; p.out_cap = s2.cap;
  if ((rc = run_viterbi(e, m, p, k.vitp, s2.vgrp))) return rc;
  CKM_CUDA(cudaEventRecord(e->ev[EV_FWD], st));
  p.in = s2.b.as<Candidate>(); p.in_count = e->d_counters + CTR_VIT; p.in_cap = s2.cap;
  p.out = s2.a.as<Candidate>(); p.out_count = e->d_counters + CTR_FWD; p.out_cap = s2.cap;
  if ((rc = per_class(e, p, launch_fwd2, 8, launch_fwd, 4, true))) return rc;
  CKM_CUDA(cudaEventRecord(e->ev[EV_CASCADE_END], st));
  e->stats.kernel_launches += 3 + (k.vitp ? N_BLK_CLASSES : 0) + (p.use_blk ? 2 * N_BLK_CLASSES : 0);
  return CKM_OK;
}

static int64_t envelope_need(const ckm_models *m, const PairWork &pw, const Envelope &en, bool use_blk) {
  const int64_t Ld = en.j - en.i + 1, Mpad = ((m->models[pw.model].M + 1) + 31) / 32 * 32 + 32;
  const int64_t vq = use_blk ? vq_of(m->models[pw.model].M) : 0;
  const int64_t width = vq ? 32 * vq : Mpad;
  return (vq ? 1 : 2) * (Ld + 1) * 3 * width + (Ld + 1) * 15 + 64;
}
static int run_envelope_waves(ckm_engine *e, const ckm_models *m, const std::vector<PairWork> &pairs, DomdefParams &p, int64_t budget,
                              DevBuf &scratch, std::vector<Envelope> &ev, DevBuf &d_ev, DevBuf &d_ord, bool leave_last) {
  if (ev.empty()) return CKM_OK;
  cudaStream_t st = e->stream;
  int rc;
  std::vector<int64_t> need(ev.size());
  std::vector<int8_t> ecls(ev.size());
  for (size_t i = 0; i < ev.size(); ++i) {
    const PairWork &pw = pairs[ev[i].pair];
    need[i] = envelope_need(m, pw, ev[i], p.use_blk != 0);
    ecls[i] = (int8_t)cls_of(m->models[pw.model].M, p.use_blk != 0);
  }
  budget = std::max<int64_t>(budget, *std::max_element(need.begin(), need.end()));
  if ((rc = d_ev.alloc(sizeof(Envelope) * ev.size())) || (rc = d_ord.alloc(sizeof(int32_t) * ev.size()))) return rc;
  std::vector<int32_t> eorder(ev.size());
  for (size_t w0 = 0, w1; w0 < ev.size(); w0 = w1) {
    int64_t tot = 0;
    for (w1 = w0; w1 < ev.size() && (w1 == w0 || tot + need[w1] <= budget); ++w1) { ev[w1].scratch_off = tot; tot += need[w1]; }
    if (sizeof(float) * (size_t)tot > scratch.bytes && (rc = scratch.alloc(sizeof(float) * (size_t)tot))) return rc;
    for (size_t i = w0; i < w1; ++i) eorder[i] = (int32_t)i;
    std::stable_sort(eorder.begin() + w0, eorder.begin() + w1, [&](int32_t a, int32_t b) { return ecls[a] != ecls[b] ? ecls[a] > ecls[b] : need[a] > need[b]; });
    CKM_CUDA(cudaMemcpyAsync(d_ev.as<Envelope>() + w0, ev.data() + w0, sizeof(Envelope) * (w1 - w0), cudaMemcpyHostToDevice, st));
    CKM_CUDA(cudaMemcpyAsync(d_ord.as<int32_t>() + w0, eorder.data() + w0, sizeof(int32_t) * (w1 - w0), cudaMemcpyHostToDevice, st));
    p.envs = d_ev.as<Envelope>(); p.env_order = d_ord.as<int32_t>(); p.scratch = scratch.as<float>();
    if ((rc = launch_class_runs(e, eorder, ecls, w0, w1, [&](int c, int32_t b0, int32_t b1, int grid, cudaStream_t s) -> int {
          p.env_begin = b0; p.env_end = b1; return c < N_BLK_CLASSES ? launch_envelopes2(p, c, grid, s) : launch_envelopes(p, grid, s); }))) return rc;
    CKM_CUDA(cudaStreamSynchronize(st));
    if (w1 < ev.size() || !leave_last) { if ((rc = fan_in(e))) return rc; CKM_CUDA(cudaStreamSynchronize(st)); }
  }
  return CKM_OK;
}

struct QueryPlan { ActiveMasks am; bool per_bin = false; std::vector<std::vector<int32_t>> qorder; int64_t n_pairs = 0; };
static int plan_queries(const ckm_models *m, const ckm_seqdb *db, const int32_t *model_idx, int32_t nmodels, const int64_t *bin_model_offsets, QueryPlan &q, cudaStream_t st) {
  const int ndb = (int)m->models.size();
  if (model_idx == nullptr && bin_model_offsets == nullptr) nmodels = ndb;
  std::vector<int32_t> slot;
  int rc = build_masks(m, db, model_idx, nmodels, bin_model_offsets, q.am, slot, st);
  if (rc) return rc;
  q.per_bin = bin_model_offsets != nullptr;
  if (q.per_bin) {
    q.qorder.assign(db->nbins, std::vector<int32_t>(ndb, -1));
    for (int b = 0; b < db->nbins; ++b) {
      for (int64_t i = bin_model_offsets[b]; i < bin_model_offsets[b + 1]; ++i) q.qorder[b][model_idx[i]] = (int32_t)(i - bin_model_offsets[b]);
      q.n_pairs += (int64_t)db->bin_nseq[b] * (bin_model_offsets[b + 1] - bin_model_offsets[b]);
    }
  } else {
    q.qorder.emplace_back(std::move(slot));
    q.n_pairs = (int64_t)db->nseq * nmodels;
  }
  return CKM_OK;
}

static int run_cascade(ckm_engine *e, const SearchKnobs &k, const ckm_models *m, const ckm_seqdb *db, ActiveMasks &am, int64_t n_pairs, Stage1 &s1, Stage2 &s2, int32_t *ctr) {
  cudaStream_t st = e->stream;
  unsigned long long cells = 0;
  int rc;
  for (int attempt = 0; attempt < QUEUE_ATTEMPTS; ++attempt) {
    if (attempt > 0) e->stats.n_queue_retries++;
    if ((rc = run_stage1(e, k, m, db, am, std::max<int64_t>(n_pairs, 1), s1, nullptr, attempt))) return rc;
    if ((rc = run_stage2(e, k, m, db, am, s1, s2, nullptr, nullptr, nullptr, nullptr))) return rc;
    CKM_CUDA(cudaMemcpyAsync(ctr, e->d_counters, sizeof(int32_t) * CTR_N, cudaMemcpyDeviceToHost, st));
    CKM_CUDA(cudaMemcpyAsync(&cells, s1.cells.p, sizeof(cells), cudaMemcpyDeviceToHost, st));
    CKM_CUDA(cudaStreamSynchronize(st));
    const bool over = ctr[CTR_CAND] > s1.cand_cap || ctr[CTR_MSV] > s1.pass_cap || ctr[CTR_BIAS] > s2.cap || ctr[CTR_VIT] > s2.cap || ctr[CTR_FWD] > s2.cap ||
                      ctr[CTR_VREDO] > s2.cap;
    if (!over) { fill_filter_stats(e, n_pairs, ctr, cells, 5); return CKM_OK; }
    if (s1.cand_cap >= std::min<int64_t>(n_pairs, QUEUE_MAX) && s1.pass_cap >= std::min<int64_t>(n_pairs, QUEUE_MAX)) break;
  }
  set_error("candidate queue overflow in the filter cascade: more than 2^30 candidate pairs in one batch; search fewer bins per call");
  return CKM_ECAPACITY;
}

static int sorted_pairs(const ckm_seqdb *db, const Candidate *d_fwd_list, int npairs, std::vector<PairWork> &pairs, int64_t &rows) {
  std::vector<Candidate> fl((size_t)npairs);
  if (npairs) CKM_CUDA(cudaMemcpy(fl.data(), d_fwd_list, sizeof(Candidate) * fl.size(), cudaMemcpyDeviceToHost));
  std::sort(fl.begin(), fl.end(), [](const Candidate &a, const Candidate &b) { return a.seq != b.seq ? a.seq < b.seq : a.model < b.model; });
  pairs.assign((size_t)npairs, PairWork{});
  rows = 0;
  for (int i = 0; i < npairs; ++i) {
    PairWork &pw = pairs[i];
    pw.seq = fl[i].seq; pw.model = fl[i].model; pw.L = db->len[pw.seq];
    pw.first_dom = 0; pw.ndom_slots = 0; pw.fwdsc = fl[i].fwdsc; pw.filtersc = fl[i].filtersc; pw.usc = fl[i].usc;
    pw.row_off = rows; rows += pw.L + 1;
  }
  return CKM_OK;
}
struct DomainStage {
  DomdefParams p{};
  DevBuf dpairs, dxf, dxb, dvec, dtbl, dregions, dporder, ddoms, dhits, dscratch, denvs, deorder, denvs2, deorder2;
  std::vector<Region> regs;
  std::vector<DomainOut> doms; std::vector<HitOut> hout;
};
static int run_regions(ckm_engine *e, const SearchKnobs &k, const ckm_models *m, const ckm_seqdb *db, const std::vector<PairWork> &pairs, int64_t rows, DomainStage &D, Trace &tr) {
  cudaStream_t st = e->stream;
  const int npairs = (int)pairs.size();
  const size_t rws = (size_t)std::max<int64_t>(rows, 1);
  int rc;
  if ((rc = D.dpairs.alloc(sizeof(PairWork) * pairs.size())) || (rc = D.dxf.alloc(sizeof(float) * rws * X_NX_HOST)) || (rc = D.dxb.alloc(sizeof(float) * rws * X_NX_HOST)) ||
      (rc = D.dvec.alloc(sizeof(float) * rws * 4)) || (rc = D.dtbl.alloc(sizeof(float) * 16000))) return rc;
  const int region_cap = npairs * 8 + 1024;
  if ((rc = D.dregions.alloc(sizeof(Region) * (size_t)region_cap))) return rc;
  CKM_CUDA(cudaMemcpyAsync(D.dpairs.p, pairs.data(), sizeof(PairWork) * pairs.size(), cudaMemcpyHostToDevice, st));
  CKM_CUDA(cudaMemcpyAsync(D.dtbl.p, logsum_table().data(), sizeof(float) * 16000, cudaMemcpyHostToDevice, st));
  CKM_CUDA(cudaMemsetAsync(e->d_counters + CTR_ENV, 0, sizeof(int32_t), st));
  DomdefParams &p = D.p = domdef_params(m, db, k);
  p.pairs = D.dpairs.as<PairWork>(); p.npairs = npairs;
  p.xf = D.dxf.as<float>(); p.xb = D.dxb.as<float>();
  p.btot = D.dvec.as<float>(); p.etot = p.btot + rws; p.mocc = p.etot + rws; p.n2sc = p.mocc + rws;
  p.regions = D.dregions.as<Region>(); p.region_count = e->d_counters + CTR_ENV; p.region_cap = region_cap;
  p.logsum_tbl = D.dtbl.as<float>();
  std::vector<int32_t> order((size_t)npairs);
  std::vector<int8_t> pcls((size_t)npairs);
  for (int i = 0; i < npairs; ++i) { order[i] = i; pcls[i] = (int8_t)cls_of(m->models[pairs[i].model].M, p.use_blk != 0); }
  std::stable_sort(order.begin(), order.end(), [&](int32_t a, int32_t b) { return pcls[a] != pcls[b] ? pcls[a] > pcls[b] : pairs[a].L > pairs[b].L; });
  if ((rc = D.dporder.alloc(sizeof(int32_t) * order.size()))) return rc;
  CKM_CUDA(cudaMemcpyAsync(D.dporder.p, order.data(), sizeof(int32_t) * order.size(), cudaMemcpyHostToDevice, st));
  p.pair_order = D.dporder.as<int32_t>();
  if ((rc = launch_class_runs(e, order, pcls, 0, (size_t)npairs, [&](int c, int32_t b0, int32_t b1, int grid, cudaStream_t s) -> int {
        p.pair_begin = b0; p.pair_end = b1; return c < N_BLK_CLASSES ? launch_regions2(p, c, grid, s) : launch_regions(p, grid, s); }))) return rc;
  if ((rc = fan_in(e))) return rc;
  int32_t nreg = 0;
  CKM_CUDA(cudaMemcpyAsync(&nreg, e->d_counters + CTR_ENV, sizeof(int32_t), cudaMemcpyDeviceToHost, st));
  CKM_CUDA(cudaStreamSynchronize(st));
  tr.mark("regions kernels");
  if (nreg > region_cap) { set_error("region queue overflow"); return CKM_ECAPACITY; }
  D.regs.resize((size_t)nreg);
  if (nreg) CKM_CUDA(cudaMemcpy(D.regs.data(), D.dregions.p, sizeof(Region) * D.regs.size(), cudaMemcpyDeviceToHost));
  std::sort(D.regs.begin(), D.regs.end(), [](const Region &a, const Region &b) { return a.pair != b.pair ? a.pair < b.pair : a.i < b.i; });
  tr.mark("regions sorted");
  return CKM_OK;
}

struct AbandonJob { cudaStream_t st; void operator()(EnsembleJob *job) const { ensembles_abandon(job, st); } };
static int domain_pass(ckm_engine *e, const SearchKnobs &k, const ckm_models *m, std::vector<PairWork> &pairs, DomainStage &D,
                       const std::vector<int> &multi_idx, std::vector<EnsembleCaps> &caps, Trace &tr, bool *grown) {
  cudaStream_t st = e->stream;
  DomdefParams &p = D.p;
  const std::vector<Region> &regs = D.regs; const int nreg = (int)regs.size();
  int rc;
  *grown = false;
  std::vector<int32_t> reg_slot((size_t)nreg);
  std::vector<Envelope> envs1, envs2;
  int32_t nslots = 0;
  for (auto &pw : pairs) { pw.ndom_slots = 0; pw.first_dom = 0; }
  for (int r = 0, mi = 0; r < nreg; ++r) {
    PairWork &pw = pairs[regs[r].pair];
    if (pw.ndom_slots == 0) pw.first_dom = nslots;
    reg_slot[r] = nslots;
    if (!regs[r].multi) { Envelope en{}; en.pair = regs[r].pair; en.i = regs[r].i; en.j = regs[r].j; en.slot = nslots; envs1.push_back(en); }
    const int n = regs[r].multi ? caps[mi++].envelopes : 1;
    nslots += n; pw.ndom_slots += n;
  }
  D.doms.assign((size_t)nslots, DomainOut{});
  if (nslots == 0) return CKM_OK;
  if ((rc = D.ddoms.alloc(sizeof(DomainOut) * (size_t)nslots)) || (rc = D.dhits.alloc(sizeof(HitOut) * pairs.size()))) return rc;
  CKM_CUDA(cudaMemsetAsync(D.ddoms.p, 0, sizeof(DomainOut) * (size_t)nslots, st));
  CKM_CUDA(cudaMemcpyAsync(D.dpairs.p, pairs.data(), sizeof(PairWork) * pairs.size(), cudaMemcpyHostToDevice, st));
  p.doms = D.ddoms.as<DomainOut>();
  const bool multi = !multi_idx.empty();
  bool ens_first = (k.ens_first == 1);
  if (k.ens_first < 0 && multi) {
    int64_t tot = 0;
    for (const Envelope &en : envs1) tot += envelope_need(m, pairs[en.pair], en, p.use_blk != 0);
    ens_first = tot > k.env_budget;
  }
  std::unique_ptr<EnsembleJob, AbandonJob> ens(nullptr, AbandonJob{e->aux});
  auto launch_ensemble = [&]() -> int {
    CKM_CUDA(cudaEventRecord(e->fan_ev, st));
    CKM_CUDA(cudaStreamWaitEvent(e->aux, e->fan_ev, 0));
    EnsembleJob *job = nullptr;
    const int r = ensembles_launch(e, m, p, pairs, regs, multi_idx, caps, e->aux, &job);
    ens.reset(job);
    return r;
  };
  if (multi && ens_first && (rc = launch_ensemble())) return rc;
  if ((rc = run_envelope_waves(e, m, pairs, p, k.env_budget, D.dscratch, envs1, D.denvs, D.deorder, multi))) return rc;
  tr.mark("envelope batch 1 launched");
  if (multi) {
    if (!ens_first && (rc = launch_ensemble())) return rc;
    if (!envs1.empty()) { if ((rc = fan_in(e))) return rc; CKM_CUDA(cudaStreamSynchronize(st)); }
    std::vector<std::vector<Envelope>> multi_envs; std::vector<EnsembleCaps> grow;
    int n_over = 0;
    if ((rc = ensembles_collect(ens.release(), e->aux, multi_envs, grow, &n_over))) return rc;
    tr.mark("batch 1 + ensemble done");
    if (n_over > 0) {
      for (size_t mi = 0; mi < caps.size(); ++mi) if (grow[mi].segments) caps[mi] = grow[mi];
      *grown = true;
      return CKM_OK;
    }
    for (size_t mi = 0; mi < multi_idx.size(); ++mi) {
      int c = 0;
      for (Envelope en : multi_envs[mi]) { en.slot = reg_slot[multi_idx[mi]] + c++; envs2.push_back(en); }
    }
    if ((rc = run_envelope_waves(e, m, pairs, p, k.env_budget, D.dscratch, envs2, D.denvs2, D.deorder2, false))) return rc;
    tr.mark("envelope batch 2 done");
  }
  p.hits = D.dhits.as<HitOut>();
  if ((rc = launch_scores(p, ((int)pairs.size() + 127) / 128, st))) return rc;
  e->stats.kernel_launches++;
  CKM_CUDA(cudaMemcpyAsync(D.doms.data(), D.ddoms.p, sizeof(DomainOut) * D.doms.size(), cudaMemcpyDeviceToHost, st));
  CKM_CUDA(cudaMemcpyAsync(D.hout.data(), D.dhits.p, sizeof(HitOut) * D.hout.size(), cudaMemcpyDeviceToHost, st));
  CKM_CUDA(cudaStreamSynchronize(st));
  return CKM_OK;
}
constexpr int DOMAIN_PASSES = 4;
static int run_domain_phase(ckm_engine *e, const SearchKnobs &k, const ckm_models *m, std::vector<PairWork> &pairs, DomainStage &D, Trace &tr) {
  std::vector<int> multi_idx;
  for (int r = 0; r < (int)D.regs.size(); ++r) if (D.regs[r].multi) multi_idx.push_back(r);
  std::vector<EnsembleCaps> caps(multi_idx.size(), ENS_DEFAULT_CAPS);
  D.hout.assign(pairs.size(), HitOut{});
  for (int pass = 0; pass < DOMAIN_PASSES; ++pass) {
    if (pass > 0) e->stats.n_queue_retries++;
    bool grown = false;
    int rc = domain_pass(e, k, m, pairs, D, multi_idx, caps, tr, &grown);
    if (rc || !grown) return rc;
  }
  set_error("a multi-domain region keeps outgrowing the capacities it asked for");
  return CKM_ECAPACITY;
}

static std::vector<ckm_hit> assemble_rows(ckm_engine *e, const ckm_models *m, const ckm_seqdb *db, const QueryPlan &q, const std::vector<PairWork> &pairs,
                                          const std::vector<HitOut> &hout, const std::vector<DomainOut> &doms, double Ecut, double domEcut) {
  struct Key { int bin, q, pair; double lnP; int seq; };
  std::vector<Key> keys;
  for (int i = 0; i < (int)pairs.size(); ++i) {
    if (!hout[i].valid) continue;
    const int b = db->bin_of_seq[pairs[i].seq];
    keys.push_back(Key{b, (q.per_bin ? q.qorder[b] : q.qorder[0])[pairs[i].model], i, hout[i].lnP, pairs[i].seq});
  }
  std::sort(keys.begin(), keys.end(), [](const Key &a, const Key &b) {
    if (a.bin != b.bin) return a.bin < b.bin;
    if (a.q != b.q) return a.q < b.q;
    if (a.lnP != b.lnP) return a.lnP < b.lnP;
    return a.seq < b.seq;
  });
  std::vector<ckm_hit> rows_out;
  size_t g0 = 0;
  int64_t n_dom = 0;
  for (size_t i = 0; i < doms.size(); ++i) if (doms[i].ok) n_dom++;
  while (g0 < keys.size()) {
    size_t g1 = g0;
    while (g1 < keys.size() && keys[g1].bin == keys[g0].bin && keys[g1].q == keys[g0].q) ++g1;
    const double Z = (double)db->bin_nseq[keys[g0].bin];
    double domZ = 0.0;
    for (size_t k = g0; k < g1; ++k) if (std::exp(keys[k].lnP) * Z <= Ecut) domZ += 1.0;
    for (size_t k = g0; k < g1; ++k) {
      if (!(std::exp(keys[k].lnP) * Z <= Ecut)) continue;
      const PairWork &pw = pairs[keys[k].pair];
      const HitOut &h = hout[keys[k].pair];
      int nrep = 0;
      for (int d = pw.first_dom; d < pw.first_dom + pw.ndom_slots; ++d)
        if (doms[d].ok && std::exp(doms[d].lnP) * domZ <= domEcut) nrep++;
      int nd = 0;
      for (int d = pw.first_dom; d < pw.first_dom + pw.ndom_slots; ++d) {
        const DomainOut &dm = doms[d];
        if (!dm.ok || !(std::exp(dm.lnP) * domZ <= domEcut)) continue;
        ckm_hit r;
        std::memset(&r, 0, sizeof(r));
        r.bin = keys[k].bin; r.seq = pw.seq; r.model = pw.model; r.tlen = pw.L; r.qlen = m->models[pw.model].M;
        r.dom = ++nd; r.ndom = nrep;
        r.hmm_from = dm.hmmfrom; r.hmm_to = dm.hmmto; r.ali_from = dm.sqfrom; r.ali_to = dm.sqto; r.env_from = dm.ienv; r.env_to = dm.jenv;
        r.full_score = h.score; r.full_bias = h.pre_score - h.score;
        r.dom_score = dm.bitscore; r.dom_bias = (float)((double)dm.dombias * 1.44269504088896341);
        r.acc = (float)(dm.oasc / (1.0 + std::fabs((float)(dm.jenv - dm.ienv))));
        r.full_evalue = std::exp(h.lnP) * Z; r.c_evalue = std::exp(dm.lnP) * domZ; r.i_evalue = std::exp(dm.lnP) * Z;
        r.full_lnP = h.lnP; r.dom_lnP = dm.lnP;
        rows_out.push_back(r);
      }
    }
    g0 = g1;
  }
  e->stats.n_hits_seq = (int64_t)keys.size(); e->stats.n_domains = n_dom; e->stats.n_reported = (int64_t)rows_out.size();
  return rows_out;
}

static int do_search(ckm_engine *e, const SearchKnobs &k, const ckm_models *m, const int32_t *model_idx, int32_t nmodels,
                     const int64_t *bin_model_offsets, const ckm_seqdb *db, double Ecut, double domEcut, ckm_hit **hits_out, int64_t *nhits_out) {
  cudaStream_t st = e->stream;
  *hits_out = nullptr; *nhits_out = 0;
  PoolScope pool_scope(e);
  QueryPlan q;
  int rc = plan_queries(m, db, model_idx, nmodels, bin_model_offsets, q, st);
  if (rc) return rc;
  std::memset(&e->stats, 0, sizeof(e->stats));
  if (q.n_pairs > ((int64_t)1 << 40)) { set_error("ckm_search: more than 2^40 (ORF x HMM) pairs in one call; search fewer bins per call"); return CKM_ECAPACITY; }
  CKM_CUDA(cudaEventRecord(e->ev[EV_CALL], st));
  Trace tr(k.trace);
  Stage1 s1; Stage2 s2; int32_t ctr[CTR_N];
  if ((rc = run_cascade(e, k, m, db, q.am, q.n_pairs, s1, s2, ctr))) return rc;
  tr.mark("filters done");
  std::vector<PairWork> pairs; int64_t rows = 0;
  if ((rc = sorted_pairs(db, s2.a.as<Candidate>(), ctr[CTR_FWD], pairs, rows))) return rc;
  CKM_CUDA(cudaEventRecord(e->ev[EV_DOMDEF], st));
  tr.mark("pair list sorted");
  DomainStage D;
  if (!pairs.empty()) {
    if ((rc = run_regions(e, k, m, db, pairs, rows, D, tr))) return rc;
    if ((rc = run_domain_phase(e, k, m, pairs, D, tr))) return rc;
  }
  CKM_CUDA(cudaEventRecord(e->ev[EV_END], st));
  CKM_CUDA(cudaEventSynchronize(e->ev[EV_END]));
  tr.mark("scores + downloads");
  const std::vector<ckm_hit> rows_out = assemble_rows(e, m, db, q, pairs, D.hout, D.doms, Ecut, domEcut);
  tr.mark("rows assembled");
  cudaEventElapsedTime(&e->stats.ms_domdef, e->ev[EV_DOMDEF], e->ev[EV_END]);
  cudaEventElapsedTime(&e->stats.ms_total, e->ev[EV_CALL], e->ev[EV_END]);
  if (!rows_out.empty()) {
    ckm_hit *out = (ckm_hit *)std::malloc(sizeof(ckm_hit) * rows_out.size());
    if (!out) { set_error("out of host memory"); return CKM_ENOMEM; }
    std::memcpy(out, rows_out.data(), sizeof(ckm_hit) * rows_out.size());
    *hits_out = out;
  }
  *nhits_out = (int64_t)rows_out.size();
  return CKM_OK;
}

static int align_pass(ckm_engine *e, const SearchKnobs &k, const ckm_models *m, const ckm_seqdb *db, std::vector<PairWork> &pairs,
                      std::vector<Envelope> &envs, int64_t rows, std::vector<int32_t> &trace, std::vector<DomainOut> &doms) {
  cudaStream_t st = e->stream;
  PoolScope pool_scope(e);
  DevBuf dpairs, dn2, dtrace, ddoms, dscratch, denvs, deorder;
  int rc;
  const size_t rws = (size_t)rows;
  if ((rc = dpairs.alloc(sizeof(PairWork) * pairs.size())) || (rc = dn2.alloc(sizeof(float) * rws)) || (rc = dtrace.alloc(sizeof(int32_t) * rws)) ||
      (rc = ddoms.alloc(sizeof(DomainOut) * pairs.size()))) return rc;
  CKM_CUDA(cudaMemcpyAsync(dpairs.p, pairs.data(), sizeof(PairWork) * pairs.size(), cudaMemcpyHostToDevice, st));
  CKM_CUDA(cudaMemsetAsync(dn2.p, 0, sizeof(float) * rws, st));
  CKM_CUDA(cudaMemsetAsync(dtrace.p, 0, sizeof(int32_t) * rws, st));
  CKM_CUDA(cudaMemsetAsync(ddoms.p, 0, sizeof(DomainOut) * pairs.size(), st));
  DomdefParams p = domdef_params(m, db, k);
  p.pairs = dpairs.as<PairWork>(); p.npairs = (int32_t)pairs.size();
  p.n2sc = dn2.as<float>(); p.trace = dtrace.as<int32_t>();
  p.doms = ddoms.as<DomainOut>();
  if ((rc = run_envelope_waves(e, m, pairs, p, k.env_budget, dscratch, envs, denvs, deorder, false))) return rc;
  trace.resize(rws);
  doms.resize(pairs.size());
  CKM_CUDA(cudaMemcpyAsync(trace.data(), dtrace.p, sizeof(int32_t) * rws, cudaMemcpyDeviceToHost, st));
  CKM_CUDA(cudaMemcpyAsync(doms.data(), ddoms.p, sizeof(DomainOut) * doms.size(), cudaMemcpyDeviceToHost, st));
  CKM_CUDA(cudaStreamSynchronize(st));
  return CKM_OK;
}

static int do_align(ckm_engine *e, const SearchKnobs &k, const ckm_models *m, int32_t model, const ckm_seqdb *db, int32_t *state_out, float *oasc_out) {
  std::memset(&e->stats, 0, sizeof(e->stats));
  const int nseq = db->nseq;
  for (int64_t i = 0; i < db->nres; ++i) state_out[i] = 0;
  if (oasc_out) for (int s = 0; s < nseq; ++s) oasc_out[s] = 0.0f;
  std::vector<PairWork> pairs;
  std::vector<Envelope> envs;
  int64_t rows = 0;
  auto add = [&](int s, int i, int j) {
    PairWork pw{};
    pw.seq = s; pw.model = model; pw.L = db->len[s]; pw.first_dom = (int32_t)pairs.size(); pw.ndom_slots = 1; pw.row_off = rows;
    rows += pw.L + 1;
    Envelope en{};
    en.pair = (int32_t)pairs.size(); en.i = i; en.j = j; en.null2_done = 1; en.slot = (int32_t)pairs.size();
    pairs.push_back(pw); envs.push_back(en);
  };
  for (int s = 0; s < nseq; ++s) if (db->len[s] > 0) add(s, 1, db->len[s]);
  if (pairs.empty()) return CKM_OK;
  std::vector<int32_t> trace; std::vector<DomainOut> doms;
  int rc;
  if ((rc = align_pass(e, k, m, db, pairs, envs, rows, trace, doms))) return rc;
  auto emit = [&](const std::vector<PairWork> &pp, const std::vector<DomainOut> &dd, const std::vector<int32_t> &tr, std::vector<int> *failed) {
    for (size_t pi = 0; pi < pp.size(); ++pi) {
      const PairWork &pw = pp[pi];
      if (!dd[pi].ok) { if (failed) failed->push_back(pw.seq); continue; }
      if (oasc_out) oasc_out[pw.seq] = dd[pi].oasc;
      int32_t *dst = state_out + (db->offsets[pw.seq] - db->offsets[0]);
      for (int i = 1; i <= pw.L; ++i) dst[i - 1] = tr[pw.row_off + i];
    }
  };
  std::vector<int> failed;
  emit(pairs, doms, trace, &failed);
  if (failed.empty()) return CKM_OK;
  ckm_hit *hits = nullptr; int64_t nhits = 0;
  if ((rc = do_search(e, k, m, &model, 1, nullptr, db, 1e300, 1e300, &hits, &nhits))) return rc;
  std::vector<int> best(nseq, -1);
  for (int64_t h = 0; h < nhits; ++h) { const int s = hits[h].seq; if (best[s] < 0 || hits[h].dom_score > hits[best[s]].dom_score) best[s] = (int)h; }
  pairs.clear(); envs.clear(); rows = 0;
  for (int s : failed) if (best[s] >= 0) add(s, hits[best[s]].env_from, hits[best[s]].env_to);
  std::free(hits);
  if (pairs.empty()) return CKM_OK;
  if ((rc = align_pass(e, k, m, db, pairs, envs, rows, trace, doms))) return rc;
  emit(pairs, doms, trace, nullptr);
  return CKM_OK;
}

static int checked_search(ckm_engine *e, const ckm_models *m, const int32_t *model_idx, int32_t nmodels, const int64_t *bin_model_offsets,
                          const ckm_seqdb *db, double E, double domE, ckm_hit **hits_out, int64_t *nhits_out) {
  if (!e || !m || !db || !hits_out || !nhits_out) { set_error("ckm_search: bad argument"); return CKM_EINVAL; }
  cudaSetDevice(e->device);
  return do_search(e, read_knobs(true), m, model_idx, nmodels, bin_model_offsets, db, E, domE, hits_out, nhits_out);
}

}

extern "C" {

int ckm_search(ckm_engine *e, const ckm_models *m, const int32_t *model_idx, int32_t nmodels,
               const ckm_seqdb *db, double E, double domE, ckm_hit **hits_out, int64_t *nhits_out) {
  return checked_search(e, m, model_idx, nmodels, nullptr, db, E, domE, hits_out, nhits_out);
}
int ckm_search_per_bin(ckm_engine *e, const ckm_models *m, const int32_t *model_idx, const int64_t *bin_model_offsets,
                       const ckm_seqdb *db, double E, double domE, ckm_hit **hits_out, int64_t *nhits_out) {
  if (!model_idx || !bin_model_offsets) { set_error("ckm_search_per_bin: bad argument"); return CKM_EINVAL; }
  return checked_search(e, m, model_idx, 0, bin_model_offsets, db, E, domE, hits_out, nhits_out);
}
int ckm_align(ckm_engine *e, const ckm_models *m, int32_t model, const ckm_seqdb *db, int32_t *state_out, float *oasc_out) {
  if (!e || !m || !db || !state_out) { set_error("ckm_align: bad argument"); return CKM_EINVAL; }
  if (model < 0 || model >= (int)m->models.size()) { set_error("ckm_align: model index out of range"); return CKM_EINVAL; }
  cudaSetDevice(e->device);
  return do_align(e, read_knobs(true), m, model, db, state_out, oasc_out);
}

int ckm_write_domtblout(const ckm_models *m, const ckm_hit *hits, int64_t nhits, int32_t bin, int32_t seq_base,
                        const char *const *names, const char *const *descs, const char *path) {
  if (!m || (!hits && nhits > 0) || !names || !path) { set_error("ckm_write_domtblout: bad argument"); return CKM_EINVAL; }
  FILE *fp = std::fopen(path, "w");
  if (!fp) { set_error(std::string("cannot write ") + path); return CKM_EIO; }
  int tnamew = 20, qnamew = 20, qaccw = 10, taccw = 10;
  for (int64_t i = 0; i < nhits; ++i) {
    if (hits[i].bin != bin) continue;
    const Model &md = m->models[hits[i].model];
    tnamew = std::max<int>(tnamew, (int)std::strlen(names[hits[i].seq - seq_base]));
    qnamew = std::max<int>(qnamew, (int)md.name.size());
    qaccw = std::max<int>(qaccw, (int)md.acc.size());
  }
  std::fprintf(fp, "#%*s %22s %40s %11s %11s %11s\n", tnamew + qnamew - 1 + 15 + taccw + qaccw, "", "--- full sequence ---",
               "-------------- this domain -------------", "hmm coord", "ali coord", "env coord");
  std::fprintf(fp, "#%-*s %-*s %5s %-*s %-*s %5s %9s %6s %5s %3s %3s %9s %9s %6s %5s %5s %5s %5s %5s %5s %5s %4s %s\n",
               tnamew - 1, " target name", taccw, "accession", "tlen", qnamew, "query name", qaccw, "accession", "qlen",
               "E-value", "score", "bias", "#", "of", "c-Evalue", "i-Evalue", "score", "bias", "from", "to", "from", "to", "from", "to", "acc", "description of target");
  std::fprintf(fp, "#%*s %*s ----- %*s %*s ----- --------- ------ ----- --- --- --------- --------- ------ ----- ----- ----- ----- ----- ----- ----- ---- ---------------------\n",
               tnamew - 1, "-------------------", taccw, "----------", qnamew, "--------------------", qaccw, "----------");
  for (int64_t i = 0; i < nhits; ++i) {
    const ckm_hit &h = hits[i];
    if (h.bin != bin) continue;
    const Model &md = m->models[h.model];
    const char *desc = (descs && descs[h.seq - seq_base] && descs[h.seq - seq_base][0]) ? descs[h.seq - seq_base] : "-";
    std::fprintf(fp, "%-*s %-*s %5d %-*s %-*s %5d %9.2g %6.1f %5.1f %3d %3d %9.2g %9.2g %6.1f %5.1f %5d %5d %5d %5d %5d %5d %4.2f %s\n",
                 tnamew, names[h.seq - seq_base], taccw, "-", h.tlen, qnamew, md.name.c_str(), qaccw, md.acc.empty() ? "-" : md.acc.c_str(), h.qlen,
                 h.full_evalue, h.full_score, h.full_bias, h.dom, h.ndom, h.c_evalue, h.i_evalue, h.dom_score, h.dom_bias,
                 h.hmm_from, h.hmm_to, h.ali_from, h.ali_to, h.env_from, h.env_to, h.acc, desc);
  }
  std::fprintf(fp, "#\n# Program:         checkm_b200 (libckm.so)\n# Pipeline mode:   SEARCH\n# [ok]\n");
  std::fclose(fp);
  return CKM_OK;
}

int ckm_filter_scores(ckm_engine *e, const ckm_models *m, const int32_t *model_idx, int32_t nmodels,
                      const ckm_seqdb *db, float *filtersc_out, float *vit_out, float *fwd_out, uint8_t *passed_out) {
  if (!e || !m || !db || !filtersc_out || !vit_out || !fwd_out || !passed_out) { set_error("ckm_filter_scores: bad argument"); return CKM_EINVAL; }
  cudaSetDevice(e->device);
  const SearchKnobs k = read_knobs(false);
  PoolScope pool_scope(e);
  QueryPlan q;
  int rc = plan_queries(m, db, model_idx, nmodels, nullptr, q, e->stream);
  if (rc) return rc;
  const int64_t n = q.n_pairs;
  DevBuf dfs, dvit, dfwd, dpass;
  const size_t nf = (size_t)std::max<int64_t>(n, 1);
  if ((rc = dfs.alloc(sizeof(float) * nf)) || (rc = dvit.alloc(sizeof(float) * nf)) || (rc = dfwd.alloc(sizeof(float) * nf)) ||
      (rc = dpass.alloc(nf + 4))) return rc;
  for (DevBuf *b : {&dfs, &dvit, &dfwd}) CKM_CUDA(cudaMemsetAsync(b->p, 0xff, sizeof(float) * nf, e->stream));
  CKM_CUDA(cudaMemsetAsync(dpass.p, 0, nf + 4, e->stream));
  Stage1 s1; Stage2 s2;
  std::memset(&e->stats, 0, sizeof(e->stats));
  if ((rc = run_stage1(e, k, m, db, q.am, n, s1, nullptr))) return rc;
  if ((rc = run_stage2(e, k, m, db, q.am, s1, s2, dfs.as<float>(), dvit.as<float>(), dfwd.as<float>(), dpass.as<uint8_t>()))) return rc;
  int32_t ctr[CTR_N];
  CKM_CUDA(cudaMemcpyAsync(ctr, e->d_counters, sizeof(ctr), cudaMemcpyDeviceToHost, e->stream));
  CKM_CUDA(cudaMemcpyAsync(filtersc_out, dfs.p, sizeof(float) * (size_t)n, cudaMemcpyDeviceToHost, e->stream));
  CKM_CUDA(cudaMemcpyAsync(vit_out, dvit.p, sizeof(float) * (size_t)n, cudaMemcpyDeviceToHost, e->stream));
  CKM_CUDA(cudaMemcpyAsync(fwd_out, dfwd.p, sizeof(float) * (size_t)n, cudaMemcpyDeviceToHost, e->stream));
  CKM_CUDA(cudaMemcpyAsync(passed_out, dpass.p, (size_t)n, cudaMemcpyDeviceToHost, e->stream));
  CKM_CUDA(cudaStreamSynchronize(e->stream));
  if (ctr[CTR_CAND] > s1.cand_cap || ctr[CTR_MSV] > s1.pass_cap) { set_error("candidate queue overflow"); return CKM_ECAPACITY; }
  std::vector<Candidate> pass1((size_t)ctr[CTR_MSV]);
  if (!pass1.empty()) CKM_CUDA(cudaMemcpy(pass1.data(), s1.pass.p, sizeof(Candidate) * pass1.size(), cudaMemcpyDeviceToHost));
  for (const Candidate &c : pass1) passed_out[(int64_t)q.qorder[0][c.model] * db->nseq + c.seq] |= 1;
  fill_filter_stats(e, n, ctr,  0, 5);
  return CKM_OK;
}

int ckm_viterbi_scores(ckm_engine *e, const ckm_models *m, const int32_t *model_idx, int32_t nmodels,
                       const ckm_seqdb *db, int32_t mode, float *vit_out) {
  if (!e || !m || !db || !vit_out) { set_error("ckm_viterbi_scores: bad argument"); return CKM_EINVAL; }
  cudaSetDevice(e->device);
  cudaStream_t st = e->stream;
  const int ndb = (int)m->models.size();
  if (model_idx == nullptr) nmodels = ndb;
  const int64_t n = (int64_t)nmodels * db->nseq;
  if (n > ((int64_t)1 << 30)) { set_error("ckm_viterbi_scores: too many pairs for one call"); return CKM_ECAPACITY; }
  PoolScope pool_scope(e);
  ActiveMasks am; std::vector<int32_t> slot;
  int rc = build_masks(m, db, model_idx, nmodels, nullptr, am, slot, st);
  if (rc) return rc;
  std::vector<int32_t> slot_model((size_t)std::max(nmodels, 1));
  for (int i = 0; i < nmodels; ++i) slot_model[i] = model_idx ? model_idx[i] : i;
  const size_t nf = (size_t)std::max<int64_t>(n, 1);
  DevBuf dsm, din, dout, dredo, dvit, dgrp;
  if ((rc = dsm.alloc(sizeof(int32_t) * slot_model.size())) || (rc = din.alloc(sizeof(Candidate) * nf)) || (rc = dout.alloc(sizeof(Candidate) * nf)) ||
      (rc = dredo.alloc(sizeof(Candidate) * nf)) || (rc = dvit.alloc(sizeof(float) * nf))) return rc;
  CKM_CUDA(cudaMemcpyAsync(dsm.p, slot_model.data(), sizeof(int32_t) * slot_model.size(), cudaMemcpyHostToDevice, st));
  CKM_CUDA(cudaMemsetAsync(e->d_counters, 0, CTR_N * sizeof(int32_t), st));
  CKM_CUDA(cudaMemsetAsync(dvit.p, 0xff, sizeof(float) * nf, st));
  std::memset(&e->stats, 0, sizeof(e->stats));
  if (n > 0) {
    if ((rc = launch_all_pairs(din.as<Candidate>(), e->d_counters + CTR_BIAS, dsm.as<int32_t>(), nmodels, db->nseq, st))) return rc;
    FilterParams p = filter_params(m, db, am);
    p.use_blk = (mode == 2) ? 0 : 1;
    p.dense_vit = dvit.as<float>();
    p.redo = dredo.as<Candidate>(); p.redo_count = e->d_counters + CTR_VREDO; p.redo_cap = (int32_t)nf;
    p.in = din.as<Candidate>(); p.in_count = e->d_counters + CTR_BIAS; p.in_cap = (int32_t)nf;
    p.out = dout.as<Candidate>(); p.out_count = e->d_counters + CTR_VIT; p.out_cap = (int32_t)nf;
    if ((rc = run_viterbi(e, m, p, mode == 0, dgrp))) return rc;
  }
  int32_t ctr[CTR_N];
  CKM_CUDA(cudaMemcpyAsync(ctr, e->d_counters, sizeof(ctr), cudaMemcpyDeviceToHost, st));
  CKM_CUDA(cudaMemcpyAsync(vit_out, dvit.p, sizeof(float) * (size_t)n, cudaMemcpyDeviceToHost, st));
  CKM_CUDA(cudaStreamSynchronize(st));
  e->stats.n_pairs = n; e->stats.n_past_bias = ctr[CTR_BIAS]; e->stats.n_past_vit = ctr[CTR_VIT]; e->stats.n_vit_redo = ctr[CTR_VREDO];
  return CKM_OK;
}

int ckm_msv_scores(ckm_engine *e, const ckm_models *m, const int32_t *model_idx, int32_t nmodels,
                   const ckm_seqdb *db, int32_t *xj_out) {
  if (!e || !m || !db || !xj_out) { set_error("ckm_msv_scores: bad argument"); return CKM_EINVAL; }
  cudaSetDevice(e->device);
  const SearchKnobs k = read_knobs(false);
  PoolScope pool_scope(e);
  QueryPlan q;
  int rc = plan_queries(m, db, model_idx, nmodels, nullptr, q, e->stream);
  if (rc) return rc;
  const int64_t n = q.n_pairs;
  DevBuf dense;
  if ((rc = dense.alloc(sizeof(int32_t) * (size_t)std::max<int64_t>(n, 1)))) return rc;
  CKM_CUDA(cudaMemsetAsync(dense.p, 0xff, sizeof(int32_t) * (size_t)n, e->stream));
  Stage1 s1;
  std::memset(&e->stats, 0, sizeof(e->stats));
  if ((rc = run_stage1(e, k, m, db, q.am, n, s1, dense.as<int32_t>()))) return rc;
  int32_t ctr[CTR_N];
  CKM_CUDA(cudaMemcpyAsync(ctr, e->d_counters, sizeof(ctr), cudaMemcpyDeviceToHost, e->stream));
  unsigned long long cells = 0;
  CKM_CUDA(cudaMemcpyAsync(&cells, s1.cells.p, sizeof(cells), cudaMemcpyDeviceToHost, e->stream));
  CKM_CUDA(cudaMemcpyAsync(xj_out, dense.p, sizeof(int32_t) * (size_t)n, cudaMemcpyDeviceToHost, e->stream));
  CKM_CUDA(cudaStreamSynchronize(e->stream));
  if (ctr[CTR_CAND] > s1.cand_cap || ctr[CTR_MSV] > s1.pass_cap) { set_error("candidate queue overflow"); return CKM_ECAPACITY; }
  fill_filter_stats(e, n, ctr, cells, 2);
  return CKM_OK;
}

}
```

checkm_b200/csrc/stages.hpp:

```cpp
#pragma once
#include "engine.hpp"

namespace ckm {

#ifndef CKM_SSV_WARPS
#define CKM_SSV_WARPS 16
#endif
constexpr int SSV_WARPS = CKM_SSV_WARPS;
constexpr int SSV_WARPS_HOST = SSV_WARPS;
constexpr int MSV_WARPS = 8;

struct SsvParams {
  const uint8_t *res; const int64_t *off; const int32_t *len; const int32_t *bin;
  const float *msvB; const int32_t *tjb; const int32_t *order;
  int32_t nseq, seq_chunk, nchunks;
  const TileGroup *groups; const int32_t *group_list; int32_t ngroups;
  const TileDesc *tiles; const TileModel *tile_models;
  const int32_t *chain_first_tile, *chain_ntiles;
  const uint8_t *tile_blob;
  const uint8_t *tile_active;
  const uint8_t *model_active;
  int32_t ntiles, nmodels;
  int32_t *unit_counter;
  int2 *cand; int32_t *cand_count; int32_t cand_cap;
  int16_t *bnd; int64_t bnd_stride;
  unsigned long long *cells;
  int32_t resolve;
  const ModelScalars *ms; const float *nullsc;
  Candidate *pass; int32_t *pass_count; int32_t pass_cap;
  int32_t *resolved_count;
  int32_t *xj_dense; const int32_t *model_slot;
  double F1;
};

int launch_ssv(int J, const SsvParams &p, int grid, size_t smem_bytes, cudaStream_t stream);

struct MsvParams {
  const uint8_t *res; const int64_t *off; const int32_t *len;
  const float *nullsc; const int32_t *tjb;
  const ModelScalars *ms; const uint8_t *rbv; const uint32_t *rmb;
  const int2 *cand; const int32_t *cand_count; int32_t cand_cap;
  Candidate *out; int32_t *out_count; int32_t out_cap;
  int32_t *xj_dense;
  const int32_t *model_slot;
  int32_t nseq;
  int32_t row_bytes;
  int32_t use_blk;
  double F1;
};

int launch_msv_exact(const MsvParams &p, int grid, cudaStream_t stream);
int launch_ssv_bypass(const int32_t *models, int32_t nbypass, int32_t nseq, const int32_t *len, const int32_t *bin,
                      const uint8_t *model_active, int32_t nmodels_db, int2 *cand, int32_t *cand_count, int32_t cand_cap,
                      cudaStream_t stream);
int launch_msv2(const MsvParams &p, int cls, int grid, cudaStream_t stream);

constexpr int VIT_WARPS = 4;
constexpr int FWD_WARPS = 4;
struct FilterParams {
  const uint8_t *res; const int64_t *off; const int32_t *len;
  const float *lenA, *lenB;
  const int16_t *tmove_w;
  const ModelScalars *ms;
  const float *bias_eo; const int16_t *rwv; const int16_t *twv; const float *rfv; const float *tfv;
  const uint4 *twb; const uint32_t *rwb; const float4 *tfb; const float *rfb;
  const uint4 *twp; const uint32_t *rwp;
  Candidate *redo; int32_t *redo_count; int32_t redo_cap;
  int32_t *vit_idx; int2 *vit_chunks; int32_t *vit_cls_chunks; int32_t *vit_work;
  const Candidate *in; const int32_t *in_count; int32_t in_cap;
  Candidate *out; int32_t *out_count; int32_t out_cap;
  int32_t row_elems;
  double F1, F2, F3;
  int32_t use_blk;
  float *dense_filtersc, *dense_vit, *dense_fwd; uint8_t *dense_passed;
  const int32_t *model_slot; int32_t nseq;
};
int launch_bias(const FilterParams &p, int grid, cudaStream_t st);
int launch_vit(const FilterParams &p, int grid, cudaStream_t st);
constexpr int N_BLK_CLASSES = 10;
constexpr int BLK_Q[N_BLK_CLASSES] = {2, 4, 6, 8, 12, 16, 20, 24, 28, 32};
int launch_vit2(const FilterParams &p, int cls, int grid, cudaStream_t st);
int launch_vitp(const FilterParams &p, int cls, int grid, cudaStream_t st);
constexpr int VITP_CHUNK = 64;
int launch_vit_group(const FilterParams &p, int32_t nmodels, int32_t *ws, int grid, cudaStream_t st);
int launch_all_pairs(Candidate *out, int32_t *count, const int32_t *slot_model, int32_t nslots, int32_t nseq, cudaStream_t st);
int launch_fwd(const FilterParams &p, int grid, cudaStream_t st);

#define FLT_MIN_F 1.17549435e-38f
struct PairWork {
  int32_t seq, model, L;
  int32_t first_dom, ndom_slots;
  float   fwdsc, filtersc, usc;
  int64_t row_off;
};
struct Region { int32_t pair, i, j, multi; };
constexpr int ENS_MAXENV = 32;
struct EnsembleCaps { int32_t segments, trace_segments, envelopes; };
constexpr EnsembleCaps ENS_DEFAULT_CAPS = {4096, 64, ENS_MAXENV};
struct Envelope { int32_t pair, i, j, null2_done; int64_t scratch_off; int32_t slot, pad; };
struct DomainOut {
  int32_t pair, ienv, jenv, hmmfrom, hmmto, sqfrom, sqto, ok;
  float   envsc, domcorrection, oasc, bitscore, dombias, pad;
  double  lnP;
};
struct HitOut { float pre_score, score, sum_score; int32_t ndom, valid, pad; double lnP; };
struct DomdefParams {
  const uint8_t *res; const int64_t *off; const float *nullsc;
  const ModelScalars *ms; const float *rfv; const float *tfv;
  const PairWork *pairs; int32_t npairs;
  const int32_t *pair_order; int32_t pair_begin, pair_end;
  float *xf, *xb, *btot, *etot, *mocc, *n2sc;
  int32_t *trace;
  Region *regions; int32_t *region_count; int32_t region_cap;
  const Envelope *envs; const int32_t *env_order; int32_t env_begin, env_end;
  float *scratch;
  DomainOut *doms; HitOut *hits;
  const float *logsum_tbl;
  int32_t row_elems;
  const float4 *tfb; const float *rfb;
  int32_t use_blk;
};
int launch_regions(const DomdefParams &p, int grid, cudaStream_t st);
int launch_envelopes(const DomdefParams &p, int grid, cudaStream_t st);
int launch_scores(const DomdefParams &p, int grid, cudaStream_t st);
int launch_fwd2(const FilterParams &p, int cls, int grid, cudaStream_t st);
int launch_regions2(const DomdefParams &p, int cls, int grid, cudaStream_t st);
int launch_envelopes2(const DomdefParams &p, int cls, int grid, cudaStream_t st);

}
```

Before: 35290.

## Group envelopes by model and stage emission tables in shared memory for large models

For large model classes (Q>=24), envelopes are sorted by model and split into chunks of up to 16 same-model items. Each block stages the full emission table and transitions into shared memory once per chunk, then hands out items to warps through a dynamic atomic cursor. Emissions are then read from shared memory at the point of use instead of through global __ldg loads. The host also plans all waves up front with a single upload, launches classes in reverse order, and caps grids to resident occupancy for envelope and region kernels. This adds block-level synchronization and larger shared memory per block, which may lower occupancy.

```diff
diff --git a/checkm_b200/csrc/fwdback_blk.cuh b/checkm_b200/csrc/fwdback_blk.cuh
--- a/checkm_b200/csrc/fwdback_blk.cuh
+++ b/checkm_b200/csrc/fwdback_blk.cuh
@@ -7,7 +7,7 @@
 
 constexpr int BLK_LOOKAHEAD_MAXQ = 16;
 
-template <int Q, bool TSMEM>
+template <int Q, bool TSMEM, bool ESMEM = false>
 struct BlkModel {
   int M;
   const float *rfb;
@@ -16,6 +16,8 @@
   int lane;
   __device__ __forceinline__ float4 T0(int q) const { return TSMEM ? tsm[q * 32 + lane] : t0[TSMEM ? 0 : q]; }
   __device__ __forceinline__ float4 T1(int q) const { return TSMEM ? tsm[(Q + q) * 32 + lane] : t1[TSMEM ? 0 : q]; }
+  __device__ __forceinline__ const float *erow(int x) const { return rfb + (size_t)x * Q * 32; }
+  __device__ __forceinline__ float E(const float *row, int q) const { return ESMEM ? row[q * 32] : __ldg(row + q * 32); }
 };
 
 template <int Q, bool TSMEM>
@@ -35,8 +37,31 @@
   }
 }
 
-template <int Q, bool TSMEM, bool FULL, bool STORE_D = true>
-__device__ __forceinline__ float forward_blk(const BlkModel<Q, TSMEM> &bm, const uint8_t *__restrict__ res, int L, const Specials sp,
+template <int Q, bool TSMEM>
+__device__ __forceinline__ void blk_model_stage(const ModelScalars &ms, const float4 *tfb, const float *rfb, float *esm, float4 *tsm) {
+  const float4 *esrc = reinterpret_cast<const float4 *>(rfb + ms.blk_off * 32 * KPAD);
+  float4 *edst = reinterpret_cast<float4 *>(esm);
+  for (int z = threadIdx.x; z < KPAD * Q * 8; z += blockDim.x) edst[z] = __ldg(esrc + z);
+  if (TSMEM) {
+    const float4 *tsrc = tfb + ms.blk_off * 32 * 2;
+    for (int z = threadIdx.x; z < Q * 64; z += blockDim.x) tsm[(z & 1) * (Q * 32) + (z >> 1)] = __ldg(tsrc + z);
+  }
+}
+template <int Q, bool TSMEM>
+__device__ __forceinline__ void blk_model_bind(BlkModel<Q, TSMEM, true> &bm, const ModelScalars &ms, const float4 *tfb, const float *esm,
+                                               const float4 *tsm, int lane) {
+  bm.M = ms.M; bm.lane = lane;
+  bm.rfb = esm + lane;
+  bm.tsm = tsm;
+  if (!TSMEM) {
+    const float4 *src = tfb + ms.blk_off * 32 * 2;
+#pragma unroll
+    for (int q = 0; q < Q; ++q) { bm.t0[TSMEM ? 0 : q] = __ldg(src + (q * 32 + lane) * 2); bm.t1[TSMEM ? 0 : q] = __ldg(src + (q * 32 + lane) * 2 + 1); }
+  }
+}
+
+template <int Q, bool TSMEM, bool FULL, bool STORE_D = true, bool ESMEM>
+__device__ __forceinline__ float forward_blk(const BlkModel<Q, TSMEM, ESMEM> &bm, const uint8_t *__restrict__ res, int L, const Specials sp,
                                              float *xmx, float *full) {
   const int lane = bm.lane;
   float Mx[Q], Ix[Q], Dx[Q];
@@ -49,25 +74,30 @@
   float xE = 0.0f, xN = 1.0f, xJ = 0.0f, xB = sp.nmove, xC = 0.0f, totscale = 0.0f;
   if (xmx != nullptr && lane == 0) { xmx[X_E] = xE; xmx[X_N] = xN; xmx[X_J] = xJ; xmx[X_B] = xB; xmx[X_C] = xC; xmx[X_SCALE] = 1.0f; }
   constexpr bool LA = (Q <= BLK_LOOKAHEAD_MAXQ);
-  float ecur[Q];
+  constexpr bool AT_USE = ESMEM && !LA;
+  float ecur[AT_USE ? 1 : Q];
+  const float *erow = bm.rfb;
   int xnext;
   if (LA) {
-    const float *rp = bm.rfb + (size_t)((L >= 1) ? __ldg(res) : 0) * Q * 32;
-#pragma unroll
-    for (int q = 0; q < Q; ++q) ecur[q] = __ldg(rp + q * 32);
+    const float *rp = bm.erow((L >= 1) ? __ldg(res) : 0);
+#pragma unroll
+    for (int q = 0; q < Q; ++q) ecur[AT_USE ? 0 : q] = bm.E(rp, q);
     xnext = (L >= 2) ? __ldg(res + 1) : 0;
   } else xnext = (L >= 1) ? __ldg(res) : 0;
   for (int i = 1; i <= L; ++i) {
     float enext[LA ? Q : 1];
     {
-      const float *rp = bm.rfb + (size_t)xnext * Q * 32;
+      const float *rp = bm.erow(xnext);
       if (LA) {
 #pragma unroll
-        for (int q = 0; q < Q; ++q) enext[LA ? q : 0] = __ldg(rp + q * 32);
+        for (int q = 0; q < Q; ++q) enext[LA ? q : 0] = bm.E(rp, q);
         xnext = (i + 2 <= L) ? __ldg(res + i + 1) : 0;
       } else {
-#pragma unroll
-        for (int q = 0; q < Q; ++q) ecur[q] = __ldg(rp + q * 32);
+        if (AT_USE) erow = rp;
+        else {
+#pragma unroll
+          for (int q = 0; q < Q; ++q) ecur[AT_USE ? 0 : q] = bm.E(rp, q);
+        }
         xnext = (i + 1 <= L) ? __ldg(res + i) : 0;
       }
     }
@@ -82,7 +112,7 @@
       sv += pm * t0.y;
       sv += pi * t0.z;
       sv += pd * t0.w;
-      sv *= ecur[q];
+      sv *= AT_USE ? bm.E(erow, q) : ecur[AT_USE ? 0 : q];
       const float nI = Mx[q] * t1.y + Ix[q] * t1.z;
       md[q] = sv * t1.x;
       Mx[q] = sv; Ix[q] = nI;
@@ -132,15 +162,15 @@
     }
     if (LA) {
 #pragma unroll
-      for (int q = 0; q < Q; ++q) ecur[q] = enext[LA ? q : 0];
+      for (int q = 0; q < Q; ++q) ecur[AT_USE ? 0 : q] = enext[LA ? q : 0];
     }
   }
   return totscale + (float)log((double)(xC * sp.nmove));
 }
 
 __device__ __forceinline__ void prefetch_l2(const void *p) { asm volatile("prefetch.global.L2 [%0];" ::"l"(p)); }
-template <int Q, bool TSMEM, int MODE>
-__device__ __forceinline__ void backward_blk(const BlkModel<Q, TSMEM> &bm, const uint8_t *__restrict__ res, int L, const Specials sp,
+template <int Q, bool TSMEM, int MODE, bool ESMEM>
+__device__ __forceinline__ void backward_blk(const BlkModel<Q, TSMEM, ESMEM> &bm, const uint8_t *__restrict__ res, int L, const Specials sp,
                                              const float *fxmx, float *bxmx, float *full) {
   const int lane = bm.lane, M = bm.M;
   float Mx[Q], Ix[Q], Dx[Q];
@@ -148,21 +178,26 @@
   for (int q = 0; q < Q; ++q) { Mx[q] = 0.0f; Ix[q] = 0.0f; Dx[q] = 0.0f; }
   float xC = 0.0f, xE = 0.0f, xJ = 0.0f, xN = 0.0f, xB = 0.0f;
   constexpr bool LA = (Q <= BLK_LOOKAHEAD_MAXQ);
-  float ecur[Q];
-#pragma unroll
-  for (int q = 0; q < Q; ++q) ecur[q] = 0.0f;
+  constexpr bool AT_USE = ESMEM && !LA;
+  float ecur[AT_USE ? 1 : Q];
+#pragma unroll
+  for (int q = 0; q < (AT_USE ? 1 : Q); ++q) ecur[q] = 0.0f;
+  const float *erow = bm.rfb;
   int xnext = (L >= 1) ? __ldg(res + L - 1) : 0;
   for (int i = L; i >= 0; --i) {
     float enext[LA ? Q : 1];
     if (LA) {
-      const float *rp = bm.rfb + (size_t)xnext * Q * 32;
-#pragma unroll
-      for (int q = 0; q < Q; ++q) enext[LA ? q : 0] = __ldg(rp + q * 32);
+      const float *rp = bm.erow(xnext);
+#pragma unroll
+      for (int q = 0; q < Q; ++q) enext[LA ? q : 0] = bm.E(rp, q);
       xnext = (i >= 2) ? __ldg(res + i - 2) : 0;
     } else if (i < L) {
-      const float *rp = bm.rfb + (size_t)xnext * Q * 32;
-#pragma unroll
-      for (int q = 0; q < Q; ++q) ecur[q] = __ldg(rp + q * 32);
+      const float *rp = bm.erow(xnext);
+      if (AT_USE) erow = rp;
+      else {
+#pragma unroll
+        for (int q = 0; q < Q; ++q) ecur[AT_USE ? 0 : q] = bm.E(rp, q);
+      }
       xnext = (i >= 1) ? __ldg(res + i - 1) : 0;
     }
     if (MODE == 2 && i >= 3) {
@@ -177,7 +212,7 @@
     } else {
       float part = 0.0f;
 #pragma unroll
-      for (int q = 0; q < Q; ++q) { em[q] = Mx[q] * ecur[q]; part += em[q] * bm.T0(q).x; }
+      for (int q = 0; q < Q; ++q) { em[q] = Mx[q] * (AT_USE ? bm.E(erow, q) : ecur[AT_USE ? 0 : q]); part += em[q] * bm.T0(q).x; }
       xB = warp_sum_float(part);
       xC = xC * sp.nloop;
       xJ = (xB * sp.nmove) + (xJ * sp.nloop);
@@ -259,9 +294,9 @@
     }
     if (LA) {
 #pragma unroll
-      for (int q = 0; q < Q; ++q) ecur[q] = enext[LA ? q : 0];
-    }
-  }
-}
-
-}
+      for (int q = 0; q < Q; ++q) ecur[AT_USE ? 0 : q] = enext[LA ? q : 0];
+    }
+  }
+}
+
+}
diff --git a/checkm_b200/csrc/kernels_blk.cu b/checkm_b200/csrc/kernels_blk.cu
--- a/checkm_b200/csrc/kernels_blk.cu
+++ b/checkm_b200/csrc/kernels_blk.cu
@@ -10,6 +10,42 @@
 constexpr int BLK_WARPS = 4;
 
 template <int Q> __host__ __device__ constexpr size_t blk_tsm_bytes() { return (size_t)Q * 32 * 2 * sizeof(float4); }
+template <int Q> __host__ __device__ constexpr size_t blk_esm_bytes() { return (size_t)KPAD * Q * 32 * sizeof(float); }
+constexpr int BLKG_WARPS = 8;
+template <int Q> __host__ __device__ constexpr int env_warps() { return blk_grouped(Q) ? BLKG_WARPS : BLK_WARPS; }
+template <int Q> __host__ __device__ constexpr size_t env_smem_bytes() {
+  return (blk_grouped(Q) ? blk_esm_bytes<Q>() + blk_tsm_bytes<Q>() : (Q >= 12 ? BLK_WARPS * blk_tsm_bytes<Q>() : 0)) + env_warps<Q>() * 32 * sizeof(float);
+}
+
+template <int Q, bool TSMEM, class ModelOf, class Item>
+__device__ __forceinline__ void blk_chunks(const DomdefParams &p, float *esm, float4 *tsm, ModelOf model_of, Item item) {
+  __shared__ int s_chunk, s_next;
+  __shared__ ModelScalars s_ms;
+  const int lane = threadIdx.x & 31;
+  for (;;) {
+    __syncthreads();
+    if (threadIdx.x == 0) {
+      const int k = atomicAdd(p.cursor, 1);
+      s_chunk = k;
+      if (k < p.nchunks) { s_next = p.chunks[k].x; s_ms = p.ms[model_of(s_next)]; }
+    }
+    __syncthreads();
+    const int k = s_chunk;
+    if (k >= p.nchunks) break;
+    const int end = p.chunks[k].y;
+    blk_model_stage<Q, TSMEM>(s_ms, p.tfb, p.rfb, esm, tsm);
+    __syncthreads();
+    BlkModel<Q, TSMEM, true> bm;
+    blk_model_bind<Q, TSMEM>(bm, s_ms, p.tfb, esm, tsm, lane);
+    for (;;) {
+      int j = 0;
+      if (lane == 0) j = atomicAdd(&s_next, 1);
+      j = __shfl_sync(0xffffffffu, j, 0);
+      if (j >= end) break;
+      item(bm, s_ms, j);
+    }
+  }
+}
 
 template <int Q, bool TSMEM>
 __global__ void __launch_bounds__(BLK_WARPS * 32) fwd2_kernel(FilterParams p) {
@@ -65,21 +101,31 @@
   }
 }
 
-template <int Q, bool TSMEM>
-__global__ void __launch_bounds__(BLK_WARPS * 32) envelope2_kernel(DomdefParams p) {
+template <int Q, bool TSMEM, class ModelOf, class Item>
+__device__ __forceinline__ void env_warp_items(const DomdefParams &p, float4 *tsm, ModelOf model_of, Item item) {
+  const int lane = threadIdx.x & 31, warp = threadIdx.x >> 5;
+  for (int idx = p.env_begin + blockIdx.x * BLK_WARPS + warp; idx < p.env_end; idx += gridDim.x * BLK_WARPS) {
+    const ModelScalars ms = p.ms[model_of(idx)];
+    if (ms.vq != Q) continue;
+    BlkModel<Q, TSMEM> bm;
+    blk_model_load<Q, TSMEM>(bm, ms, p.tfb, p.rfb, tsm, lane);
+    item(bm, ms, idx);
+  }
+}
+
+template <int Q, bool TSMEM>
+__global__ void __launch_bounds__(env_warps<Q>() * 32) envelope2_kernel(DomdefParams p) {
   extern __shared__ __align__(16) uint8_t bsm[];
-  const int lane = threadIdx.x & 31, warp = threadIdx.x >> 5;
-  float4 *tsm = reinterpret_cast<float4 *>(bsm) + (size_t)warp * Q * 32 * 2;
-  float *null2 = reinterpret_cast<float *>(bsm + (TSMEM ? BLK_WARPS * blk_tsm_bytes<Q>() : 0)) + warp * 32;
+  const int warp = threadIdx.x >> 5;
+  constexpr bool GROUPED = blk_grouped(Q);
+  float *null2 = reinterpret_cast<float *>(bsm + env_smem_bytes<Q>()) - (env_warps<Q>() - warp) * 32;
   constexpr int QW = Q * 32;
-  for (int idx = p.env_begin + blockIdx.x * BLK_WARPS + warp; idx < p.env_end; idx += gridDim.x * BLK_WARPS) {
+  auto model_of = [&](int j) { return p.pairs[p.envs[p.env_order[j]].pair].model; };
+  auto body = [&](const auto &bm, const ModelScalars &ms, int idx) {
+    const int lane = bm.lane;
     const int ei = p.env_order[idx];
     const Envelope env = p.envs[ei];
     const PairWork pw = p.pairs[env.pair];
-    const ModelScalars ms = p.ms[pw.model];
-    if (ms.vq != Q) continue;
-    BlkModel<Q, TSMEM> bm;
-    blk_model_load<Q, TSMEM>(bm, ms, p.tfb, p.rfb, tsm, lane);
     const int M = ms.M, Ld = env.j - env.i + 1;
     const uint8_t *res = p.res + p.off[pw.seq] + (env.i - 1);
     const Specials sp = make_specials(pw.L, false);
@@ -137,10 +183,10 @@
       xn = __shfl_sync(0xffffffffu, xn, 0) * norm; xc = __shfl_sync(0xffffffffu, xc, 0) * norm; xj = __shfl_sync(0xffffffffu, xj, 0) * norm;
       const float xfactor = xn + xc + xj;
       for (int x = 0; x < K; ++x) {
-        const float *rp = bm.rfb + (size_t)x * QW;
+        const float *rp = bm.erow(x);
         float part = 0.0f;
 #pragma unroll
-        for (int q = 0; q < Q; ++q) { part += em[q] * __ldg(rp + q * 32); part += ein[q]; }
+        for (int q = 0; q < Q; ++q) { part += em[q] * bm.E(rp, q); part += ein[q]; }
         part = warp_sum_float(part);
         if (lane == 0) null2[x] = part + xfactor;
       }
@@ -335,41 +381,61 @@
       p.doms[env.slot] = out;
     }
     __syncwarp();
-  }
-}
-
-template <int Q, bool TSMEM, class P, class KF>
-static int launch_one(KF kern, const P &p, int grid, size_t extra, cudaStream_t st, const char *what) {
-  const size_t smem = (TSMEM ? BLK_WARPS * blk_tsm_bytes<Q>() : 0) + extra;
+  };
+  if constexpr (GROUPED) {
+    blk_chunks<Q, TSMEM>(p, reinterpret_cast<float *>(bsm), reinterpret_cast<float4 *>(bsm + blk_esm_bytes<Q>()), model_of, body);
+  } else {
+    env_warp_items<Q, TSMEM>(p, reinterpret_cast<float4 *>(bsm) + (size_t)warp * Q * 32 * 2, model_of, body);
+  }
+}
+
+template <class P, class KF>
+static int launch_kernel(KF kern, const P &p, int grid, int threads, size_t smem, cudaStream_t st, const char *what, bool resident = false) {
+  cudaError_t e;
   if (smem > 48 * 1024) {
-    cudaError_t e = cudaFuncSetAttribute(kern, cudaFuncAttributeMaxDynamicSharedMemorySize, (int)smem);
+    e = cudaFuncSetAttribute(kern, cudaFuncAttributeMaxDynamicSharedMemorySize, (int)smem);
     if (e != cudaSuccess) return cuda_fail(e, what);
   }
-  kern<<<grid, BLK_WARPS * 32, smem, st>>>(p);
-  cudaError_t e = cudaGetLastError();
+  if (resident) {
+    int dev = 0, nsm = 0, per_sm = 0;
+    if ((e = cudaGetDevice(&dev)) != cudaSuccess || (e = cudaDeviceGetAttribute(&nsm, cudaDevAttrMultiProcessorCount, dev)) != cudaSuccess ||
+        (e = cudaOccupancyMaxActiveBlocksPerMultiprocessor(&per_sm, kern, threads, smem)) != cudaSuccess) return cuda_fail(e, what);
+    if (per_sm > 0) grid = std::min(grid, nsm * per_sm);
+  }
+  kern<<<grid, threads, smem, st>>>(p);
+  e = cudaGetLastError();
   return e == cudaSuccess ? CKM_OK : cuda_fail(e, what);
 }
-
-#define CKM_CLASS_SWITCH(KERN, EXTRA, WHAT)                                                              \
+template <int Q, bool TSMEM>
+static int launch_fwd2_q(const FilterParams &p, int grid, cudaStream_t st) {
+  return launch_kernel(fwd2_kernel<Q, TSMEM>, p, grid, BLK_WARPS * 32, TSMEM ? BLK_WARPS * blk_tsm_bytes<Q>() : 0, st, "fwd2_kernel");
+}
+template <int Q, bool TSMEM>
+static int launch_regions2_q(const DomdefParams &p, int grid, cudaStream_t st) {
+  return launch_kernel(regions2_kernel<Q, TSMEM>, p, grid, BLK_WARPS * 32, TSMEM ? BLK_WARPS * blk_tsm_bytes<Q>() : 0, st, "regions2_kernel", true);
+}
+template <int Q, bool TSMEM>
+static int launch_envelopes2_q(const DomdefParams &p, int grid, cudaStream_t st) {
+  return launch_kernel(envelope2_kernel<Q, TSMEM>, p, grid, env_warps<Q>() * 32, env_smem_bytes<Q>(), st, "envelope2_kernel", true);
+}
+
+#define CKM_CLASS_SWITCH(LAUNCH, WHAT)                                                                   \
   switch (cls) {                                                                                        \
-    case 0: return launch_one<2, false>(KERN<2, false>, p, grid, EXTRA, st, WHAT);                      \
-    case 1: return launch_one<4, false>(KERN<4, false>, p, grid, EXTRA, st, WHAT);                      \
-    case 2: return launch_one<6, false>(KERN<6, false>, p, grid, EXTRA, st, WHAT);                      \
-    case 3: return launch_one<8, false>(KERN<8, false>, p, grid, EXTRA, st, WHAT);                      \
-    case 4: return launch_one<12, true>(KERN<12, true>, p, grid, EXTRA, st, WHAT);                      \
-    case 5: return launch_one<16, true>(KERN<16, true>, p, grid, EXTRA, st, WHAT);                      \
-    case 6: return launch_one<20, true>(KERN<20, true>, p, grid, EXTRA, st, WHAT);                      \
-    case 7: return launch_one<24, true>(KERN<24, true>, p, grid, EXTRA, st, WHAT);                      \
-    case 8: return launch_one<28, true>(KERN<28, true>, p, grid, EXTRA, st, WHAT);                      \
-    case 9: return launch_one<32, true>(KERN<32, true>, p, grid, EXTRA, st, WHAT);                      \
+    case 0: return LAUNCH<2, false>(p, grid, st);                                                       \
+    case 1: return LAUNCH<4, false>(p, grid, st);                                                       \
+    case 2: return LAUNCH<6, false>(p, grid, st);                                                       \
+    case 3: return LAUNCH<8, false>(p, grid, st);                                                       \
+    case 4: return LAUNCH<12, true>(p, grid, st);                                                       \
+    case 5: return LAUNCH<16, true>(p, grid, st);                                                       \
+    case 6: return LAUNCH<20, true>(p, grid, st);                                                       \
+    case 7: return LAUNCH<24, true>(p, grid, st);                                                       \
+    case 8: return LAUNCH<28, true>(p, grid, st);                                                       \
+    case 9: return LAUNCH<32, true>(p, grid, st);                                                       \
   }                                                                                                     \
   set_error(WHAT ": bad class"); return CKM_EINVAL;
 
-int launch_fwd2(const FilterParams &p, int cls, int grid, cudaStream_t st) { CKM_CLASS_SWITCH(fwd2_kernel, 0, "fwd2_kernel") }
-int launch_regions2(const DomdefParams &p, int cls, int grid, cudaStream_t st) { CKM_CLASS_SWITCH(regions2_kernel, 0, "regions2_kernel") }
-int launch_envelopes2(const DomdefParams &p, int cls, int grid, cudaStream_t st) {
-  const size_t extra = BLK_WARPS * 32 * sizeof(float);
-  CKM_CLASS_SWITCH(envelope2_kernel, extra, "envelope2_kernel")
-}
-
-}
+int launch_fwd2(const FilterParams &p, int cls, int grid, cudaStream_t st) { CKM_CLASS_SWITCH(launch_fwd2_q, "fwd2_kernel") }
+int launch_regions2(const DomdefParams &p, int cls, int grid, cudaStream_t st) { CKM_CLASS_SWITCH(launch_regions2_q, "regions2_kernel") }
+int launch_envelopes2(const DomdefParams &p, int cls, int grid, cudaStream_t st) { CKM_CLASS_SWITCH(launch_envelopes2_q, "envelope2_kernel") }
+
+}
diff --git a/checkm_b200/csrc/kernels_ensemble.cu b/checkm_b200/csrc/kernels_ensemble.cu
--- a/checkm_b200/csrc/kernels_ensemble.cu
+++ b/checkm_b200/csrc/kernels_ensemble.cu
@@ -427,14 +427,14 @@
   e->stats.kernel_launches++;
   job->envs.resize((size_t)nenv);
   job->cnt.resize(nm); job->need.resize((size_t)3 * nm);
-  CKM_CUDA(cudaMemcpyAsync(job->envs.data(), job->b_env.p, sizeof(Envelope) * job->envs.size(), cudaMemcpyDeviceToHost, st));
-  CKM_CUDA(cudaMemcpyAsync(job->cnt.data(), job->b_cnt.p, sizeof(int32_t) * nm, cudaMemcpyDeviceToHost, st));
-  CKM_CUDA(cudaMemcpyAsync(job->need.data(), job->b_need.p, sizeof(int32_t) * 3 * nm, cudaMemcpyDeviceToHost, st));
   return CKM_OK;
 }
 
 int ensembles_collect(EnsembleJob *job, cudaStream_t st, std::vector<std::vector<Envelope>> &out, std::vector<EnsembleCaps> &grow, int *n_over) {
-  cudaError_t err = cudaStreamSynchronize(st);
+  cudaError_t err = cudaMemcpyAsync(job->envs.data(), job->b_env.p, sizeof(Envelope) * job->envs.size(), cudaMemcpyDeviceToHost, st);
+  if (err == cudaSuccess) err = cudaMemcpyAsync(job->cnt.data(), job->b_cnt.p, sizeof(int32_t) * job->cnt.size(), cudaMemcpyDeviceToHost, st);
+  if (err == cudaSuccess) err = cudaMemcpyAsync(job->need.data(), job->b_need.p, sizeof(int32_t) * job->need.size(), cudaMemcpyDeviceToHost, st);
+  if (err == cudaSuccess) err = cudaStreamSynchronize(st);
   *n_over = 0;
   if (err == cudaSuccess) {
     out.assign((size_t)job->nm, {});
diff --git a/checkm_b200/csrc/search.cu b/checkm_b200/csrc/search.cu
--- a/checkm_b200/csrc/search.cu
+++ b/checkm_b200/csrc/search.cu
@@ -98,19 +98,53 @@
   }
   return fan_in(e);
 }
-template <class Launch> static int launch_class_runs(ckm_engine *e, const std::vector<int32_t> &order, const std::vector<int8_t> &cls, size_t b0, size_t b1, Launch launch) {
+static bool grouped_class(int c) { return c < N_BLK_CLASSES && blk_grouped(BLK_Q[c]); }
+struct ClassRun { int32_t ib = 0, ie = 0, cb = 0, ce = 0; };
+template <class Work>
+static void plan_runs(const std::vector<int32_t> &order, const std::vector<int8_t> &cls, const std::vector<int32_t> &model, Work work,
+                      size_t b0, size_t b1, bool group, std::vector<int2> &chunks, ClassRun *runs) {
+  for (int c = 0; c < ckm_engine::NCLS; ++c) runs[c] = ClassRun{};
+  for (size_t i = b0, r1; i < b1; i = r1) {
+    const int c = cls[order[i]];
+    for (r1 = i; r1 < b1 && cls[order[r1]] == c; ++r1) {}
+    ClassRun &r = runs[c];
+    r.ib = (int32_t)i; r.ie = (int32_t)r1; r.cb = (int32_t)chunks.size();
+    if (group && grouped_class(c)) {
+      for (size_t a = i, z; a < r1; a = z) {
+        for (z = a; z < r1 && z - a < (size_t)BLK_CHUNK && model[order[z]] == model[order[a]]; ++z) {}
+        chunks.push_back(make_int2((int32_t)a, (int32_t)z));
+      }
+      std::stable_sort(chunks.begin() + r.cb, chunks.end(), [&](int2 x, int2 y) { return work(order[x.x]) > work(order[y.x]); });
+    }
+    r.ce = (int32_t)chunks.size();
+  }
+}
+template <class Launch> static int launch_runs(ckm_engine *e, const ClassRun *runs, Launch launch) {
   const int nsm = e->prop.multiProcessorCount;
   int rc;
   if ((rc = fan_out(e))) return rc;
-  while (b0 < b1) {
-    size_t r1 = b0; const int c = cls[order[b0]];
-    while (r1 < b1 && cls[order[r1]] == c) ++r1;
-    const int cnt = (int)(r1 - b0);
-    const int grid = c < N_BLK_CLASSES ? std::min(nsm * 8, (cnt + 3) / 4) : std::min(nsm * 4, (cnt + FWD_WARPS - 1) / FWD_WARPS);
-    if ((rc = launch(c, (int32_t)b0, (int32_t)r1, grid, e->cls[c]))) return rc;
+  for (int c = ckm_engine::NCLS - 1; c >= 0; --c) {
+    const ClassRun &r = runs[c];
+    if (r.ie <= r.ib) continue;
+    const int n = r.ie - r.ib;
+    const int grid = r.ce > r.cb ? std::min(nsm * 8, r.ce - r.cb) : c < N_BLK_CLASSES ? std::min(nsm * 8, (n + 3) / 4) : std::min(nsm * 4, (n + FWD_WARPS - 1) / FWD_WARPS);
+    if ((rc = launch(c, r, grid, e->cls[c]))) return rc;
     e->stats.kernel_launches++;
-    b0 = r1;
-  }
+  }
+  return CKM_OK;
+}
+static int upload_plan(DevBuf &buf, const std::vector<int2> &chunks, const std::vector<int32_t> &order, size_t ncursors, cudaStream_t st,
+                       const int2 **d_chunks, const int32_t **d_order, int32_t **d_cursors) {
+  const size_t cb = sizeof(int2) * chunks.size(), ob = sizeof(int32_t) * order.size();
+  int rc;
+  if ((rc = buf.alloc(cb + ob + sizeof(int32_t) * ncursors))) return rc;
+  uint8_t *base = static_cast<uint8_t *>(buf.p);
+  if (cb) CKM_CUDA(cudaMemcpyAsync(base, chunks.data(), cb, cudaMemcpyHostToDevice, st));
+  if (ob) CKM_CUDA(cudaMemcpyAsync(base + cb, order.data(), ob, cudaMemcpyHostToDevice, st));
+  CKM_CUDA(cudaMemsetAsync(base + cb + ob, 0, sizeof(int32_t) * ncursors, st));
+  *d_chunks = reinterpret_cast<const int2 *>(base);
+  *d_order = reinterpret_cast<const int32_t *>(base + cb);
+  *d_cursors = reinterpret_cast<int32_t *>(base + cb + ob);
   return CKM_OK;
 }
 
@@ -357,22 +391,36 @@
     ecls[i] = (int8_t)cls_of(m->models[pw.model].M, p.use_blk != 0);
   }
   budget = std::max<int64_t>(budget, *std::max_element(need.begin(), need.end()));
-  if ((rc = d_ev.alloc(sizeof(Envelope) * ev.size())) || (rc = d_ord.alloc(sizeof(int32_t) * ev.size()))) return rc;
-  std::vector<int32_t> eorder(ev.size());
+  std::vector<int32_t> eorder(ev.size()), emodel(ev.size());
+  std::vector<int2> chunks;
+  std::vector<size_t> wave_end;
+  std::vector<ClassRun> runs;
+  int64_t scratch_max = 0;
+  for (size_t i = 0; i < ev.size(); ++i) { eorder[i] = (int32_t)i; emodel[i] = pairs[ev[i].pair].model; }
   for (size_t w0 = 0, w1; w0 < ev.size(); w0 = w1) {
     int64_t tot = 0;
     for (w1 = w0; w1 < ev.size() && (w1 == w0 || tot + need[w1] <= budget); ++w1) { ev[w1].scratch_off = tot; tot += need[w1]; }
-    if (sizeof(float) * (size_t)tot > scratch.bytes && (rc = scratch.alloc(sizeof(float) * (size_t)tot))) return rc;
-    for (size_t i = w0; i < w1; ++i) eorder[i] = (int32_t)i;
-    std::stable_sort(eorder.begin() + w0, eorder.begin() + w1, [&](int32_t a, int32_t b) { return ecls[a] != ecls[b] ? ecls[a] > ecls[b] : need[a] > need[b]; });
-    CKM_CUDA(cudaMemcpyAsync(d_ev.as<Envelope>() + w0, ev.data() + w0, sizeof(Envelope) * (w1 - w0), cudaMemcpyHostToDevice, st));
-    CKM_CUDA(cudaMemcpyAsync(d_ord.as<int32_t>() + w0, eorder.data() + w0, sizeof(int32_t) * (w1 - w0), cudaMemcpyHostToDevice, st));
-    p.envs = d_ev.as<Envelope>(); p.env_order = d_ord.as<int32_t>(); p.scratch = scratch.as<float>();
-    if ((rc = launch_class_runs(e, eorder, ecls, w0, w1, [&](int c, int32_t b0, int32_t b1, int grid, cudaStream_t s) -> int {
-          p.env_begin = b0; p.env_end = b1; return c < N_BLK_CLASSES ? launch_envelopes2(p, c, grid, s) : launch_envelopes(p, grid, s); }))) return rc;
-    CKM_CUDA(cudaStreamSynchronize(st));
-    if (w1 < ev.size() || !leave_last) { if ((rc = fan_in(e))) return rc; CKM_CUDA(cudaStreamSynchronize(st)); }
-  }
+    scratch_max = std::max(scratch_max, tot);
+    std::stable_sort(eorder.begin() + w0, eorder.begin() + w1, [&](int32_t a, int32_t b) {
+      return ecls[a] != ecls[b] ? ecls[a] > ecls[b] : grouped_class(ecls[a]) && emodel[a] != emodel[b] ? emodel[a] < emodel[b] : need[a] > need[b]; });
+    runs.resize(runs.size() + ckm_engine::NCLS);
+    plan_runs(eorder, ecls, emodel, [&](int32_t i) { return need[i]; }, w0, w1, true, chunks, runs.data() + runs.size() - ckm_engine::NCLS);
+    wave_end.push_back(w1);
+  }
+  if (sizeof(float) * (size_t)scratch_max > scratch.bytes && (rc = scratch.alloc(sizeof(float) * (size_t)scratch_max))) return rc;
+  if ((rc = d_ev.alloc(sizeof(Envelope) * ev.size()))) return rc;
+  CKM_CUDA(cudaMemcpyAsync(d_ev.p, ev.data(), sizeof(Envelope) * ev.size(), cudaMemcpyHostToDevice, st));
+  const int2 *d_chunks; const int32_t *d_order; int32_t *d_cursors;
+  if ((rc = upload_plan(d_ord, chunks, eorder, runs.size(), st, &d_chunks, &d_order, &d_cursors))) return rc;
+  p.envs = d_ev.as<Envelope>(); p.env_order = d_order; p.scratch = scratch.as<float>();
+  for (size_t w = 0; w < wave_end.size(); ++w) {
+    if ((rc = launch_runs(e, runs.data() + w * ckm_engine::NCLS, [&](int c, const ClassRun &r, int grid, cudaStream_t s) -> int {
+          p.env_begin = r.ib; p.env_end = r.ie;
+          p.chunks = d_chunks + r.cb; p.nchunks = r.ce - r.cb; p.cursor = d_cursors + w * ckm_engine::NCLS + c;
+          return c < N_BLK_CLASSES ? launch_envelopes2(p, c, grid, s) : launch_envelopes(p, grid, s); }))) return rc;
+    if (w + 1 < wave_end.size() || !leave_last) { if ((rc = fan_in(e))) return rc; CKM_CUDA(cudaStreamSynchronize(st)); }
+  }
+  CKM_CUDA(cudaStreamSynchronize(st));
   return CKM_OK;
 }
 
@@ -459,11 +507,14 @@
   std::vector<int8_t> pcls((size_t)npairs);
   for (int i = 0; i < npairs; ++i) { order[i] = i; pcls[i] = (int8_t)cls_of(m->models[pairs[i].model].M, p.use_blk != 0); }
   std::stable_sort(order.begin(), order.end(), [&](int32_t a, int32_t b) { return pcls[a] != pcls[b] ? pcls[a] > pcls[b] : pairs[a].L > pairs[b].L; });
+  std::vector<int2> no_chunks;
+  ClassRun runs[ckm_engine::NCLS];
+  plan_runs(order, pcls, {}, [](int32_t) { return 0; }, 0, (size_t)npairs, false, no_chunks, runs);
   if ((rc = D.dporder.alloc(sizeof(int32_t) * order.size()))) return rc;
   CKM_CUDA(cudaMemcpyAsync(D.dporder.p, order.data(), sizeof(int32_t) * order.size(), cudaMemcpyHostToDevice, st));
   p.pair_order = D.dporder.as<int32_t>();
-  if ((rc = launch_class_runs(e, order, pcls, 0, (size_t)npairs, [&](int c, int32_t b0, int32_t b1, int grid, cudaStream_t s) -> int {
-        p.pair_begin = b0; p.pair_end = b1; return c < N_BLK_CLASSES ? launch_regions2(p, c, grid, s) : launch_regions(p, grid, s); }))) return rc;
+  if ((rc = launch_runs(e, runs, [&](int c, const ClassRun &r, int grid, cudaStream_t s) -> int {
+        p.pair_begin = r.ib; p.pair_end = r.ie; return c < N_BLK_CLASSES ? launch_regions2(p, c, grid, s) : launch_regions(p, grid, s); }))) return rc;
   if ((rc = fan_in(e))) return rc;
   int32_t nreg = 0;
   CKM_CUDA(cudaMemcpyAsync(&nreg, e->d_counters + CTR_ENV, sizeof(int32_t), cudaMemcpyDeviceToHost, st));
diff --git a/checkm_b200/csrc/stages.hpp b/checkm_b200/csrc/stages.hpp
--- a/checkm_b200/csrc/stages.hpp
+++ b/checkm_b200/csrc/stages.hpp
@@ -119,7 +119,10 @@
   int32_t row_elems;
   const float4 *tfb; const float *rfb;
   int32_t use_blk;
+  const int2 *chunks; int32_t nchunks; int32_t *cursor;
 };
+__host__ __device__ constexpr bool blk_grouped(int Q) { return Q >= 24; }
+constexpr int BLK_CHUNK = 16;
 int launch_regions(const DomdefParams &p, int grid, cudaStream_t st);
 int launch_envelopes(const DomdefParams &p, int grid, cudaStream_t st);
 int launch_scores(const DomdefParams &p, int grid, cudaStream_t st);
```

Result: faster. 35760 (median of 6 runs) (+1.3%).
